# mayuelala/FollowYourClick

Measured on AMD Instinct MI355X. Metric: denoised frames/sec, 16f x 512^2 clip @ 25 DDIM steps, higher is better.
Workload: dtype bf16; 1 GPU; configs[1]: AnimationPipeline DDIM loop, SD-1.5 UNet3D + mm_sd_v15-shaped motion modules (random init), 1 clip/GPU of 16 frames 512x512, 25 DDIM steps, CFG 8.0, mask + first-frame concat, fps/flow conditioning; frames=16, height=512, width=512, ddim_steps=25, parallelism=dp1 (independent clips, weight broadcast 0.00 GiB in 0.00s)

## Files before the change

### followyourclick_amd/_build.py

```python
import concurrent.futures as cf
import hashlib
import os
import shutil
import subprocess
import sys

HERE = os.path.dirname(os.path.abspath(__file__))
CSRC = os.path.join(HERE, "csrc")
EXTRA = os.environ.get("FYC_BUILD_EXTRA", "").split()
LIB = os.path.abspath(os.environ.get("FYC_BUILD_LIB") or os.path.join(HERE, "libfyc_hip.so"))
OBJ = os.path.join(HERE, "_obj") if not (EXTRA or os.environ.get("FYC_BUILD_LIB")) else LIB + ".obj"
SOURCES = ["api.hip", "gemm.hip", "gemm_bf16_plain.hip", "gemm_bf16_conv.hip", "gemm_bf16_act.hip", "gemm_f16_plain.hip", "gemm_f16_conv.hip", "gemm_f16_act.hip", "gemm_f32.hip", "attention.hip", "attention_small.hip", "attention_medium.hip", "attention_large.hip", "attention_small_f16.hip", "attention_medium_f16.hip", "attention_large_f16.hip", "temporal_attn.hip", "temporal_block.hip", "temporal_block_rr.hip", "ff_block.hip", "panel_linear.hip", "norm.hip", "elementwise.hip"]
VARIANTS = os.environ.get("FYC_GEMM_VARIANTS") == "1"
VARIANT_DIR = os.path.join(HERE, "..", "tools", "exp", "gemm_variants")
VARIANT_SOURCES = ["gemm_pp_plain.hip", "gemm_pp_conv.hip", "gemm_ov.hip"] if VARIANTS else []
if VARIANTS:
    EXTRA = EXTRA + ["-DFYC_GEMM_VARIANTS"]
    if not os.environ.get("FYC_BUILD_LIB"):
        raise SystemExit("FYC_GEMM_VARIANTS=1 needs FYC_BUILD_LIB=<path>: the experiment kernels are not part of the product library")
FLAGS = ["--offload-arch=gfx950", "-O3", "-std=c++17", "-fPIC", "-ffp-contract=off", "-Wno-unused-value",
         "-mllvm", "-amdgpu-mfma-vgpr-form=1"]
AGPR_SOURCES = {"ff_block.hip", "panel_linear.hip", "temporal_block_rr.hip"}


NO_SLP_SOURCES = set(filter(None, os.environ.get("FYC_NO_SLP", "ff_block.hip").split(",")))


NO_NAN_SOURCES = {s for s in SOURCES if s.startswith("attention")}


def _flags(src: str):
    fl = FLAGS
    if src in AGPR_SOURCES:
        fl = [f for f in FLAGS if f not in ("-mllvm", "-amdgpu-mfma-vgpr-form=1")]
    if src in NO_SLP_SOURCES:
        fl = fl + ["-fno-slp-vectorize"]
    if src in NO_NAN_SOURCES and os.environ.get("FYC_ATTN_HONOR_NANS") != "1":
        fl = fl + ["-fno-honor-nans"]
    return fl + EXTRA


def _hipcc() -> str:
    for c in (os.environ.get("HIPCC"), shutil.which("hipcc"), "/opt/rocm/bin/hipcc"):
        if c and os.path.exists(c):
            return c
    raise RuntimeError("hipcc not found (need ROCm with gfx950 support)")


def _digest(path: str) -> str:
    h = hashlib.sha256()
    for dep in [path, os.path.join(CSRC, "fyc_common.h"), os.path.join(CSRC, "gemm_kernel.h"), os.path.join(CSRC, "attention_kernel.h"), os.path.join(CSRC, "attention_groups.h"), os.path.join(HERE, "..", "include", "fyc.h")]:
        with open(dep, "rb") as f:
            h.update(f.read())
    h.update(" ".join(_flags(os.path.basename(path))).encode())
    return h.hexdigest()


def source_digest() -> str:
    h = hashlib.sha256()
    files = sorted(f for f in os.listdir(CSRC) if f.endswith((".hip", ".h")))
    for f in files:
        h.update(f.encode())
        with open(os.path.join(CSRC, f), "rb") as fh:
            h.update(fh.read())
    with open(os.path.join(HERE, "..", "include", "fyc.h"), "rb") as fh:
        h.update(fh.read())
    for src in SOURCES:
        h.update((src + " " + " ".join(_flags(src))).encode())
    return h.hexdigest()


def family_digest(family: str = "gemm") -> str:
    if family != "gemm":
        raise ValueError(family)
    h = hashlib.sha256()
    files = sorted(f for f in os.listdir(CSRC) if f.startswith("gemm") and f.endswith((".hip", ".h"))) + ["fyc_common.h"]
    for f in files:
        h.update(f.encode())
        with open(os.path.join(CSRC, f), "rb") as fh:
            h.update(fh.read())
    for src in SOURCES:
        if src.startswith("gemm"):
            h.update((src + " " + " ".join(_flags(src))).encode())
    return h.hexdigest()


def _compile(src: str) -> str:
    path = os.path.join(VARIANT_DIR if src in VARIANT_SOURCES else CSRC, src)
    obj = os.path.join(OBJ, src.replace(".hip", ".o"))
    stamp = obj + ".sha"
    dig = _digest(path)
    if os.path.exists(obj) and os.path.exists(stamp) and open(stamp).read() == dig:
        return obj
    cmd = [_hipcc(), *_flags(src), "-c", path, "-o", obj]
    r = subprocess.run(cmd, capture_output=True, text=True)
    if r.returncode != 0:
        raise RuntimeError(f"hipcc failed for {src}:\n{r.stderr[-4000:]}")
    with open(stamp, "w") as f:
        f.write(dig)
    return obj


def build(force: bool = False, verbose: bool = True) -> str:
    os.makedirs(OBJ, exist_ok=True)
    if force:
        for f in os.listdir(OBJ):
            os.remove(os.path.join(OBJ, f))
    with cf.ThreadPoolExecutor(max_workers=len(SOURCES)) as ex:
        objs = list(ex.map(_compile, SOURCES + VARIANT_SOURCES))
    newest = max(os.path.getmtime(o) for o in objs)
    if force or not os.path.exists(LIB) or os.path.getmtime(LIB) < newest:
        r = subprocess.run([_hipcc(), "--offload-arch=gfx950", "-shared", "-fPIC", "-o", LIB, *objs], capture_output=True, text=True)
        if r.returncode != 0:
            raise RuntimeError(f"link failed:\n{r.stderr[-4000:]}")
    if verbose:
        print(f"[fyc] built {LIB} ({os.path.getsize(LIB) >> 10} KiB)")
    return LIB


if __name__ == "__main__":
    build(force="--force" in sys.argv)
```

### followyourclick_amd/_lib.py

```python
from __future__ import annotations

import ctypes as C
import os

HERE = os.path.dirname(os.path.abspath(__file__))
LIB_PATH = os.environ.get("FYC_LIB_PATH") or os.path.join(HERE, "libfyc_hip.so")

FYC_F32, FYC_BF16, FYC_F16 = 0, 1, 2
GEMM_PLAIN, GEMM_CONV3X3, GEMM_CONV3X3_UP2 = 0, 1, 2
EPI_LINEAR, EPI_GEGLU, EPI_HEADS = 0, 1, 2
ACT_NONE, ACT_GELU, ACT_QUICK_GELU = 0, 1, 2

i32, i64, f32, vp = C.c_int32, C.c_int64, C.c_float, C.c_void_p


class GemmArgs(C.Structure):
    _fields_ = [("a", vp), ("a2", vp), ("w", vp), ("bias", vp), ("rowbias", vp), ("residual", vp), ("out", vp),
                ("seg_out", vp * 3), ("seg_transposed", i32 * 3), ("seg_ld", i32 * 3),
                ("M", i32), ("N", i32), ("K", i32),
                ("lda", i32), ("ldw", i32), ("ldo", i32), ("ldr", i32), ("ldrb", i32), ("k_split", i32), ("lda2", i32),
                ("stride_a", i64), ("stride_w", i64), ("stride_o", i64),
                ("batch", i32), ("mode", i32), ("epilogue", i32),
                ("Hout", i32), ("Wout", i32), ("Hin", i32), ("Win", i32), ("Cin", i32), ("conv_stride", i32), ("conv_pad", i32),
                ("rows_per_batch", i32), ("seg_cols", i32), ("heads", i32), ("tokens", i32),
                ("out_scale", f32), ("dtype", i32), ("tile", i32), ("act", i32), ("ln_stats", vp), ("ln_colsum", vp),
                ("ln_nparts", i32), ("ln_eps", f32), ("chan_parts", vp), ("cs_rows", i32), ("row_parts", vp), ("row_nparts", i32), ("workspace", vp), ("workspace_bytes", i64)]


class AttnArgs(C.Structure):
    _fields_ = [("q", vp), ("k", vp), ("vt", vp), ("o", vp),
                ("batch", i32), ("heads", i32), ("n_q", i32), ("n_k", i32), ("d", i32),
                ("ldo", i32), ("ldvt", i32), ("kv_batch_div", i32), ("o_accumulate", i32),
                ("scale", f32), ("o_scale", f32), ("dtype", i32)]


class TAttnArgs(C.Structure):
    _fields_ = [("qkv", vp), ("o", vp), ("clips", i32), ("frames", i32), ("pixels", i32), ("heads", i32), ("d", i32),
                ("scale", f32), ("dtype", i32)]


class GnStatsArgs(C.Structure):
    _fields_ = [("x", vp), ("stats", vp), ("rows", i32), ("C", i32), ("groups", i32), ("rows_per_sample", i32), ("dtype", i32),
                ("pad_", i32), ("workspace", vp), ("workspace_bytes", i64)]


class GnApplyArgs(C.Structure):
    _fields_ = [("x", vp), ("stats", vp), ("gamma", vp), ("beta", vp), ("y", vp),
                ("rows", i32), ("C", i32), ("groups", i32), ("rows_per_sample", i32), ("eps", f32), ("silu", i32), ("dtype", i32)]


class ChanStatsReduceArgs(C.Structure):
    _fields_ = [("parts", vp), ("cs", vp), ("rows", i32), ("N", i32), ("cs_rows", i32), ("tile_rows", i32), ("slots", i32), ("out_rows", i32)]


class GnApplyCsArgs(C.Structure):
    _fields_ = [("x1", vp), ("cs1", vp), ("x2", vp), ("cs2", vp), ("gamma", vp), ("beta", vp), ("y", vp),
                ("C1", i32), ("C2", i32), ("rows", i32), ("groups", i32), ("rows_per_sample", i32), ("eps", f32), ("silu", i32),
                ("dtype", i32), ("cs_rows", i32)]


class LayerNormArgs(C.Structure):
    _fields_ = [("x", vp), ("gamma", vp), ("beta", vp), ("pe", vp), ("y", vp),
                ("rows", i32), ("C", i32), ("eps", f32), ("pe_div", i32), ("pe_rows", i32), ("dtype", i32)]


class RowStatsArgs(C.Structure):
    _fields_ = [("x", vp), ("stats", vp), ("rows", i32), ("C", i32), ("eps", f32), ("dtype", i32)]


class SoftmaxArgs(C.Structure):
    _fields_ = [("x", vp), ("rows", i64), ("cols", i32), ("ld", i32), ("dtype", i32), ("causal_rows", i32)]


class ConcatArgs(C.Structure):
    _fields_ = [("a", vp), ("b", vp), ("y", vp), ("rows", i64), ("c1", i32), ("c2", i32), ("dtype", i32)]


class SiluArgs(C.Structure):
    _fields_ = [("x", vp), ("y", vp), ("n", i64)]


class CastArgs(C.Structure):
    _fields_ = [("x", vp), ("y", vp), ("rows", i64), ("cols", i32), ("ld", i32), ("dtype", i32)]


class UnetInputArgs(C.Structure):
    _fields_ = [("latents", vp), ("mask", vp), ("first", vp), ("x", vp),
                ("B", i32), ("F", i32), ("HW", i32), ("c_latent", i32), ("c_pad", i32), ("cfg_dup", i32), ("mask_frames", i32),
                ("dtype", i32), ("mode", i32)]


class CfgDdimArgs(C.Structure):
    _fields_ = [("pred", vp), ("latents", vp), ("coef", vp),
                ("B", i32), ("F", i32), ("HW", i32), ("c_latent", i32), ("ld", i32), ("cfg", i32), ("guidance", f32),
                ("pred_type", i32), ("clip_sample", i32), ("dtype", i32), ("pred_single", vp), ("video_scale", f32),
                ("variance_noise", vp), ("sigma", f32), ("clipped_model_output", i32)]


class NchwInArgs(C.Structure):
    _fields_ = [("z", vp), ("x", vp), ("N", i32), ("C", i32), ("HW", i32), ("c_pad", i32), ("scale", f32), ("dtype", i32)]


class NhwcOutArgs(C.Structure):
    _fields_ = [("x", vp), ("y", vp), ("N", i32), ("C", i32), ("HW", i32), ("ld", i32),
                ("mul", f32), ("add", f32), ("lo", f32), ("hi", f32), ("dtype", i32)]


class EmbedArgs(C.Structure):
    _fields_ = [("ids", vp), ("table", vp), ("pos", vp), ("out", vp), ("rows", i64), ("seq", i32), ("C", i32), ("vocab", i32),
                ("dtype", i32)]


class PatchifyArgs(C.Structure):
    _fields_ = [("image", vp), ("out", vp), ("B", i32), ("Cin", i32), ("H", i32), ("W", i32), ("P", i32), ("ld", i32), ("dtype", i32)]


class TemporalBlockArgs(C.Structure):
    _fields_ = [("x", vp), ("out", vp), ("w_qkv", vp), ("colsum", vp), ("bias", vp), ("pe_bias", vp), ("w_out", vp), ("b_out", vp),
                ("clips", i32), ("frames", i32), ("pixels", i32), ("heads", i32), ("d", i32), ("C", i32),
                ("scale", C.c_float), ("eps", C.c_float), ("dtype", i32), ("wstream", vp)]


class FFBlockArgs(C.Structure):
    _fields_ = [("x", vp), ("residual", vp), ("out", vp), ("wstream", vp), ("b_out", vp), ("chan_parts", vp), ("cs_rows", i32),
                ("rows", i32), ("C", i32), ("hidden", i32), ("eps", C.c_float), ("dtype", i32)]


class PanelLinearArgs(C.Structure):
    _fields_ = [("x", vp), ("residual", vp), ("out", vp), ("wstream", vp), ("bias", vp), ("gn_cs", vp), ("gn_gamma", vp), ("gn_beta", vp),
                ("gn_rows_per_sample", i32), ("gn_stat_samples", i32), ("gn_groups", i32), ("gn_eps", C.c_float),
                ("rows", i32), ("N", i32), ("K", i32), ("dtype", i32)]


class PackConv3x3Args(C.Structure):
    _fields_ = [("w", vp), ("out", vp), ("O", i32), ("I", i32), ("dtype", i32)]


class PackGegluArgs(C.Structure):
    _fields_ = [("w", vp), ("b", vp), ("w_out", vp), ("b_out", vp), ("O", i32), ("I", i32), ("dtype", i32)]


OPS = {
    "fyc_gemm": GemmArgs, "fyc_attention": AttnArgs, "fyc_temporal_attention": TAttnArgs,
    "fyc_gn_stats": GnStatsArgs, "fyc_gn_apply": GnApplyArgs, "fyc_layernorm": LayerNormArgs,
    "fyc_softmax_rows": SoftmaxArgs, "fyc_concat_channels": ConcatArgs, "fyc_silu_f32": SiluArgs,
    "fyc_cast_from_f32": CastArgs, "fyc_cast_to_f32": CastArgs, "fyc_unet_input": UnetInputArgs,
    "fyc_cfg_ddim_step": CfgDdimArgs, "fyc_nchw_to_nhwc": NchwInArgs, "fyc_nhwc_to_nchw": NhwcOutArgs,
    "fyc_embed_tokens": EmbedArgs, "fyc_patchify": PatchifyArgs, "fyc_row_stats": RowStatsArgs,
    "fyc_gn_apply_cs": GnApplyCsArgs, "fyc_chan_stats_reduce": ChanStatsReduceArgs,
    "fyc_pack_conv3x3": PackConv3x3Args, "fyc_pack_geglu": PackGegluArgs, "fyc_temporal_block": TemporalBlockArgs,
    "fyc_ff_block": FFBlockArgs, "fyc_panel_linear": PanelLinearArgs,
}
MISC = ["fyc_version", "fyc_last_error", "fyc_init", "fyc_device_caps", "fyc_set_tuning", "fyc_gemm_row_parts", "fyc_gemm_stat_layout", "fyc_gemm_workspace_bytes", "fyc_gn_stats_workspace", "fyc_temporal_block_supported", "fyc_temporal_block_wstream_bytes",
        "fyc_ff_block_supported", "fyc_ff_block_wstream_bytes", "fyc_panel_linear_supported", "fyc_panel_linear_wstream_bytes"]

_lib = None
FYC_VERSION = 301


class FycError(RuntimeError):
    pass


def load() -> C.CDLL:
    global _lib
    if _lib is not None:
        return _lib
    if not os.path.exists(LIB_PATH):
        raise FycError(f"{LIB_PATH} is missing: build it with `python -m followyourclick_amd._build` "
                       "(hipcc --offload-arch=gfx950). There is no CPU fallback.")
    lib = C.CDLL(LIB_PATH)
    lib.fyc_version.restype = C.c_int
    ab_build = bool(os.environ.get("FYC_LIB_PATH"))
    if lib.fyc_version() != FYC_VERSION and not ab_build:
        raise FycError(f"{LIB_PATH} reports ABI version {lib.fyc_version()}, this binding was written against {FYC_VERSION}: argument structs differ "
                       "between major versions - rebuild the library (`python -m followyourclick_amd._build`)")
    lib.fyc_last_error.restype = C.c_char_p
    lib.fyc_init.argtypes = [vp]
    lib.fyc_device_caps.argtypes = [C.POINTER(i64)]
    lib.fyc_set_tuning.argtypes = [C.c_int, C.c_int]
    if not ab_build or hasattr(lib, "fyc_gemm_row_parts"):
        lib.fyc_gemm_row_parts.argtypes = [C.POINTER(GemmArgs)]
        lib.fyc_gemm_row_parts.restype = C.c_int
        lib.fyc_gemm_stat_layout.argtypes = [C.POINTER(GemmArgs), C.POINTER(i32), C.POINTER(i32)]
        lib.fyc_gemm_stat_layout.restype = C.c_int
        lib.fyc_gemm_workspace_bytes.argtypes = [C.POINTER(GemmArgs)]
        lib.fyc_gemm_workspace_bytes.restype = i64
    if not ab_build or hasattr(lib, "fyc_gn_stats_workspace"):
        lib.fyc_gn_stats_workspace.argtypes = [C.POINTER(GnStatsArgs)]
        lib.fyc_gn_stats_workspace.restype = i64
    if not ab_build or hasattr(lib, "fyc_temporal_block_supported"):
        lib.fyc_temporal_block_supported.argtypes = [C.POINTER(TemporalBlockArgs)]
        lib.fyc_temporal_block_supported.restype = C.c_int
    if not ab_build or hasattr(lib, "fyc_temporal_block_wstream_bytes"):
        lib.fyc_temporal_block_wstream_bytes.argtypes = []
        lib.fyc_temporal_block_wstream_bytes.restype = i64
    if not ab_build or hasattr(lib, "fyc_ff_block_supported"):
        lib.fyc_ff_block_supported.argtypes = [C.POINTER(FFBlockArgs)]
        lib.fyc_ff_block_supported.restype = C.c_int
        lib.fyc_ff_block_wstream_bytes.argtypes = []
        lib.fyc_ff_block_wstream_bytes.restype = i64
    if not ab_build or hasattr(lib, "fyc_panel_linear_supported"):
        lib.fyc_panel_linear_supported.argtypes = [C.POINTER(PanelLinearArgs)]
        lib.fyc_panel_linear_supported.restype = C.c_int
        lib.fyc_panel_linear_wstream_bytes.argtypes = [i32, i32]
        lib.fyc_panel_linear_wstream_bytes.restype = i64
    for name, st in OPS.items():
        if ab_build and not hasattr(lib, name):
            continue
        fn = getattr(lib, name)
        fn.argtypes = [C.POINTER(st), vp]
        fn.restype = C.c_int
    _lib = lib
    return lib


def check(rc: int, what: str) -> None:
    if rc != 0:
        raise FycError(f"{what} failed (rc={rc}): {load().fyc_last_error().decode(errors='replace')}")
```

### followyourclick_amd/engine/unet3d.py

```python
from __future__ import annotations

import math
import os
from typing import List, Optional, Sequence, Tuple, Union

import torch

from .. import _lib as L
from .. import ops as ops_mod
from .base import EngineBase
from .config import UNet3DConfig
from .weights import Packed, pack_ff_block, pack_panel_linear, pack_temporal_block

Tensor = torch.Tensor

FUSE_STATS = os.environ.get("FYC_FUSE_STATS", "1") != "0"
FUSE_TEMPORAL = os.environ.get("FYC_FUSE_TEMPORAL", "1") != "0"
TEMPORAL_RR = os.environ.get("FYC_TEMPORAL_RR", "1") != "0"
FUSE_FF = os.environ.get("FYC_FUSE_FF", "1") != "0"
FUSE_PANEL = os.environ.get("FYC_FUSE_PANEL", "1") != "0"
PANEL_ALL = os.environ.get("FYC_PANEL_ALL", "0") != "0"
FUSE_ROWS = os.environ.get("FYC_FUSE_ROWS", "0") != "0"


class Act:
    __slots__ = ("t", "C", "cs", "cs_rows", "rp", "rp_n")

    def __init__(self, t: Tensor, C: int, cs: Optional[Tensor] = None, cs_rows: int = 0, rp: Optional[Tensor] = None, rp_n: int = 0):
        self.t, self.C, self.cs, self.cs_rows, self.rp, self.rp_n = t, C, cs, cs_rows, rp, rp_n


def sinusoid_host(values: Sequence[float], dim: int) -> Tensor:
    half = dim // 2
    v = torch.tensor(list(values), dtype=torch.float32)
    freqs = torch.exp(-math.log(10000.0) * torch.arange(half, dtype=torch.float32) / half)
    ang = v[:, None] * freqs[None, :]
    return torch.cat([torch.cos(ang), torch.sin(ang)], dim=-1).contiguous()


class UNet3DEngine(EngineBase):
    def __init__(self, packed: Packed, ops=None):
        self.P = packed
        self.cfg: UNet3DConfig = packed.cfg
        self.dtype = packed.dtype
        self.ops = ops if ops is not None else ops_mod.get()
        self.device = packed.conv_in_w.device
        self.heads = self.cfg.attention_head_dim
        self.groups = self.cfg.norm_num_groups
        self.mat_attn = self.dtype == torch.float32
        self.transformers: List[Packed] = []
        for blk in self.P.down:
            self.transformers += [l.attn for l in blk.layers if l.attn is not None]
        self.transformers.append(self.P.mid.attn)
        for blk in self.P.up:
            self.transformers += [l.attn for l in blk.layers if l.attn is not None]
        for i, t in enumerate(self.transformers):
            t["idx"] = i
        self.ctx_cache = None
        self.fuse_stats = FUSE_STATS
        self.fuse_rows = FUSE_STATS and FUSE_ROWS
        self.ops.ensure_init(self.device)

    def prepare_time_embeddings(self, timesteps: Sequence[int], fps: Optional[Sequence[float]], flow: Optional[Sequence[float]],
                                batch: int, camera: Optional[Sequence[float]] = None):
        cfg, P, o = self.cfg, self.P, self.ops
        c0, S = cfg.block_out_channels[0], len(timesteps)
        rows = S * batch

        def mlp(m: Packed, sin: Tensor, residual=None) -> Tensor:
            h = self.lin(sin.to(self.device), m.w1, rows, bias=m.b1)
            a = self.new(rows, h.shape[1], dtype=torch.float32)
            o.silu_f32(h, a)
            return self.lin(a, m.w2, rows, bias=m.b2, residual=residual)

        def per_row(v):
            s = sinusoid_host(v, c0)
            return s if s.shape[0] == rows else s.repeat(S, 1)

        emb = mlp(P.emb["time_embedding"], sinusoid_host(timesteps, c0).repeat_interleave(batch, dim=0))
        if cfg.use_camera_motion_condition and camera is not None:
            emb = mlp(P.emb["camera_motion_embedding"], per_row(camera), residual=emb)
        if cfg.use_fps_condition and fps is not None:
            emb = mlp(P.emb["fps_embedding"], per_row(fps), residual=emb)
            emb = mlp(P.emb["motion_embedding"], per_row(flow), residual=emb)
        act = self.new(rows, emb.shape[1], dtype=torch.float32)
        o.silu_f32(emb, act)
        temb = self.lin(act, P.temb_w, rows, bias=P.temb_b)
        return emb, temb

    def prepare_context(self, ctx: Tensor, ip_tokens: Optional[Tensor] = None) -> None:
        cfg, o = self.cfg, self.ops
        Bn, Nk, D = ctx.shape
        H = self.heads

        def to_T(t: Tensor) -> Tensor:
            t = t.to(device=self.device, dtype=torch.float32).contiguous()
            y = self.new(t.shape[0] * t.shape[1], D)
            o.cast_from_f32(t, y, rows=t.shape[0] * t.shape[1], cols=D, ld=D)
            return y

        def project(x: Tensor, w: Tensor, n_tok: int, C: int):
            d = C // H
            ld = ((n_tok + 7) // 8) * 8
            k = self.new(Bn, H, n_tok, d)
            vt = self.zeros(Bn, H, d, ld)
            o.gemm(x, w, None, M=Bn * n_tok, N=2 * C, K=D, lda=D, ldw=D, epilogue=L.EPI_HEADS,
                   heads=dict(seg_cols=C, heads=H, tokens=n_tok, outs=[k, vt], transposed=[0, 1], ld=[0, ld]))
            return k, vt, ld

        if cfg.use_ip_cross_attention and ip_tokens is None:
            n = cfg.ip_num_tokens
            if Nk <= n:
                raise ValueError(f"encoder_hidden_states has {Nk} tokens, the IP cross-attention splits off the last {n}")
            ctx, ip_tokens = ctx[:, :Nk - n], ctx[:, Nk - n:]
            Nk -= n
        xt = to_T(ctx)
        xi = to_T(ip_tokens) if (cfg.use_ip_cross_attention and ip_tokens is not None) else None
        cache = []
        for t in self.transformers:
            e = dict(text=project(xt, t.kv2_w, Nk, t.C), n_text=Nk, ip=None)
            if xi is not None:
                e["ip"] = project(xi, t.kvip_w, ip_tokens.shape[1], t.C)
                e["n_ip"] = ip_tokens.shape[1]
            cache.append(e)
        self.ctx_cache = cache

    def _attend(self, q: Tensor, k: Tensor, vt: Tensor, out: Tensor, *, batch: int, n_q: int, n_k: int, d: int, ldvt: int,
                C: int, kv_div: int, accumulate: bool = False, o_scale: float = 1.0) -> None:
        H, o = self.heads, self.ops
        scale = d ** -0.5
        if not self.mat_attn:
            o.attention(q, k, vt, out, batch=batch, heads=H, n_q=n_q, n_k=n_k, d=d, ldo=C, ldvt=ldvt, scale=scale,
                        kv_batch_div=kv_div, accumulate=accumulate, o_scale=o_scale)
            return
        ldS = ((n_k + 7) // 8) * 8
        for b in range(batch):
            kb = b // kv_div
            S = self.zeros(H, n_q, ldS)
            o.gemm(q[b], k[kb], S, M=n_q, N=n_k, K=d, lda=d, ldw=d, ldo=ldS, batch=H, stride_a=n_q * d, stride_w=n_k * d,
                   stride_o=n_q * ldS, out_scale=scale)
            o.softmax_rows(S, rows=H * n_q, cols=n_k, ld=ldS)
            dst = out[b * n_q:(b + 1) * n_q]
            if accumulate:
                tmp = self.new(n_q, C)
                o.gemm(S, vt[kb], tmp, M=n_q, N=d, K=ldS, lda=ldS, ldw=ldvt, ldo=C, batch=H, stride_a=n_q * ldS, stride_w=d * ldvt,
                       stride_o=d)
                self._axpy(tmp, dst, n_q, C, o_scale)
            else:
                o.gemm(S, vt[kb], dst, M=n_q, N=d, K=ldS, lda=ldS, ldw=ldvt, ldo=C, batch=H, stride_a=n_q * ldS, stride_w=d * ldvt,
                       stride_o=d)

    def row_stats(self, x: Tensor, rows: int, C: int, eps: float = 1e-5) -> Tensor:
        st = self.new(rows, 2, dtype=torch.float32)
        self.ops.row_stats(x, st, rows=rows, C_=C, eps=eps)
        return st

    def _gn(self, x: Union[Act, Tuple[Act, Act]], gamma: Tensor, beta: Tensor, rows: int, rows_per_sample: int, eps: float,
            silu: bool) -> Tuple[Tensor, Optional[Tensor]]:
        o = self.ops
        if isinstance(x, Act):
            if x.cs is not None and rows_per_sample % x.cs_rows == 0:
                y = self.new(rows, x.C)
                o.gn_apply_cs(x.t, x.cs, gamma, beta, y, rows=rows, C1=x.C, groups=self.groups, rows_per_sample=rows_per_sample,
                              eps=eps, silu=silu, cs_rows=x.cs_rows)
                return y, None
            return self.group_norm(x.t, gamma, beta, rows, x.C, rows_per_sample, eps, silu), None
        a, b = x
        if a.cs is not None and b.cs is not None and a.cs_rows == b.cs_rows and rows_per_sample % a.cs_rows == 0:
            y = self.new(rows, a.C + b.C)
            o.gn_apply_cs(a.t, a.cs, gamma, beta, y, rows=rows, C1=a.C, groups=self.groups, rows_per_sample=rows_per_sample,
                          eps=eps, silu=silu, x2=b.t, cs2=b.cs, C2=b.C, cs_rows=a.cs_rows)
            return y, None
        cat = self.new(rows, a.C + b.C)
        o.concat_channels(a.t, b.t, cat, rows=rows, c1=a.C, c2=b.C)
        return self.group_norm(cat, gamma, beta, rows, a.C + b.C, rows_per_sample, eps, silu), cat

    def _lin_rp(self, x: Tensor, w: Tensor, rows: int, bias=None, residual=None) -> Act:
        N, K = w.shape
        out = self.new(rows, N, dtype=x.dtype)
        if FUSE_PANEL and PANEL_ALL and not self.fuse_rows and self.ops.panel_linear_supported(x.dtype, rows=rows, N=N, K=K):
            self.ops.panel_linear(x, out, wstream=self._panel_stream(w), rows=rows, N=N, K=K, bias=bias, residual=residual)
            return Act(out, N)
        rp, n = None, 0
        if self.fuse_rows:
            n = self.ops.gemm_row_parts(x.dtype, M=rows, N=N, K=K)
            rp = self.new(rows, n, 2, dtype=torch.float32)
        self.ops.gemm(x, w, out, M=rows, N=N, K=K, lda=K, ldw=K, ldo=N, bias=bias, residual=residual, ldr=N, row_parts=rp, row_nparts=n)
        return Act(out, N, rp=rp, rp_n=n)

    def _panel_stream(self, w: Tensor) -> Tensor:
        cache = self.__dict__.setdefault("_panel_ws", {})
        key = w.data_ptr()
        hit = cache.get(key)
        if hit is None or hit[0] is not w:
            hit = cache[key] = (w, pack_panel_linear(w))
        return hit[1]

    def _norm_proj_in(self, x: Act, node: Packed, rows: int, rows_per_sample: int) -> Act:
        C = node.C
        if (FUSE_PANEL and isinstance(x, Act) and x.cs is not None and not self.fuse_rows and rows_per_sample % x.cs_rows == 0
                and self.ops.panel_linear_supported(self.dtype, rows=rows, N=C, K=C, gn_rows_per_sample=rows_per_sample, gn_groups=self.groups)):
            out = self.new(rows, C)
            self.ops.panel_linear(x.t, out, wstream=self._panel_stream(node.pin_w), rows=rows, N=C, K=C, bias=node.pin_b, gn_cs=x.cs,
                                  gn_gamma=node.norm_g, gn_beta=node.norm_b, gn_rows_per_sample=rows_per_sample,
                                  gn_stat_samples=rows_per_sample // x.cs_rows, gn_groups=self.groups, gn_eps=1e-6)
            return Act(out, C)
        h, _ = self._gn(x, node.norm_g, node.norm_b, rows, rows_per_sample, 1e-6, False)
        return self._lin_rp(h, node.pin_w, rows, bias=node.pin_b)

    def _ln_args(self, tok: Act, rows: int, C: int) -> dict:
        if tok.rp is not None:
            return dict(ln_stats=tok.rp, ln_nparts=tok.rp_n, ln_eps=1e-5)
        return dict(ln_stats=self.row_stats(tok.t, rows, C))

    def _pe_rowbias(self, a: Packed, B: int, F: int) -> Tensor:
        key = (B, F)
        cache = a.setdefault("_pe_rb", {})
        if key not in cache:
            if F > a.pe_w.shape[0]:
                raise ValueError(f"video_length {F} exceeds the positional table ({a.pe_w.shape[0]})")
            cache[key] = a.pe_w[:F].repeat(B, 1).contiguous()
        return cache[key]

    def _axpy(self, x: Tensor, y: Tensor, rows: int, C: int, alpha: float) -> None:
        key = ("axpy", C, alpha)
        if not hasattr(self, "_eyes"):
            self._eyes = {}
        if key not in self._eyes:
            self._eyes[key] = (torch.eye(C, dtype=torch.float32) * alpha).to(self.dtype).to(self.device)
        self.ops.gemm(x, self._eyes[key], y, M=rows, N=C, K=C, lda=C, ldw=C, ldo=C, residual=y, ldr=C)

    def _conv_act(self, x: Tensor, w: Tensor, b: Tensor, frames: int, Hin: int, Win: int, nxt: Tuple[int, int], **kw) -> Act:
        Cout, K = w.shape
        if kw.get("up2"):
            Ho, Wo = kw["up_size"]
        else:
            st = kw.get("stride", 1)
            Ho, Wo = (Hin - 1) // st + 1, (Win - 1) // st + 1
        rows = frames * Ho * Wo
        plan = self._cs_plan(rows, nxt[0], Cout, K, L.GEMM_CONV3X3_UP2 if kw.get("up2") else L.GEMM_CONV3X3) if nxt else None
        out = self.conv(x, w, b, frames, Hin, Win, chan_parts=None if plan is None else plan[0], cs_rows=nxt[0] if plan is not None else 0, **kw)
        return Act(out, Cout, None if plan is None else self._cs_finish(plan, rows, nxt[0], Cout, nxt[1]), nxt[1] if nxt else 0)

    def resnet(self, r: Packed, x: Union[Act, Tuple[Act, Act]], temb: Tensor, g: dict, nxt: Tuple[int, int]) -> Act:
        rows, rpb = g["rows"], g["F"] * g["H"] * g["W"]
        frames = g["B"] * g["F"]
        h, cat = self._gn(x, r.n1_g, r.n1_b, rows, rpb, self.cfg.norm_eps, True)
        tb = temb[:, r.temb_off:]
        h1 = self._conv_act(h, r.c1_w, r.c1_b, frames, g["H"], g["W"], (g["H"] * g["W"], rpb), rowbias=tb,
                            rpb=g["H"] * g["W"] if g.get("temb_per_frame") else rpb, ldrb=temb.shape[1])
        h2, _ = self._gn(h1, r.n2_g, r.n2_b, rows, rpb, self.cfg.norm_eps, True)
        if r.sc_w is None:
            sc = x.t
        elif isinstance(x, Act) or cat is not None:
            sc = self.lin(cat if cat is not None else x.t, r.sc_w, rows, bias=r.sc_b)
        else:
            a, b = x
            sc = self.new(rows, r.cout)
            self.ops.gemm(a.t, r.sc_w, sc, M=rows, N=r.cout, K=a.C + b.C, lda=a.C, ldw=a.C + b.C, ldo=r.cout, bias=r.sc_b,
                          a2=b.t, k_split=a.C, lda2=b.C)
        return self._conv_act(h2, r.c2_w, r.c2_b, frames, g["H"], g["W"], nxt, residual=sc)

    def feed_forward_out(self, ff: Packed, ln, tok: Act, residual: Optional[Tensor], rows: int, C: int, nxt=None) -> Act:
        hidden = ff.w1.shape[0] // 2
        cs_rows = nxt[0] if (nxt and self.fuse_stats) else 0
        fused = FUSE_FF and ff.cs1 is not None
        if fused and cs_rows and not self.ops.ff_block_supported(self.dtype, rows=rows, C_=C, hidden=hidden, cs_rows=cs_rows):
            cs_rows = 0
        if fused and self.ops.ff_block_supported(self.dtype, rows=rows, C_=C, hidden=hidden, cs_rows=cs_rows):
            if "_wstream" not in ff:
                ff["_wstream"] = pack_ff_block(ff)
            out = self.new(rows, C)
            parts = self.new(rows // 128 * C * 2, dtype=torch.float32) if cs_rows else None
            self.ops.ff_block(tok.t, residual, out, wstream=ff["_wstream"], b_out=ff.po_b, rows=rows, C_=C, hidden=hidden,
                              chan_parts=parts, cs_rows=cs_rows)
            cs = self._cs_finish((parts, 128, 1), rows, nxt[0], C, nxt[1]) if cs_rows else None
            return Act(out, C, cs, nxt[1] if cs_rows else 0)
        if ff.cs1 is not None:
            N1 = ff.w1.shape[0]
            hmid = self.new(rows, N1 // 2)
            self.ops.gemm(tok.t, ff.w1, hmid, M=rows, N=N1, K=C, lda=C, ldw=C, ldo=N1 // 2, bias=ff.b1, epilogue=L.EPI_GEGLU,
                          ln_colsum=ff.cs1, **self._ln_args(tok, rows, C))
        else:
            n = self.layer_norm(tok.t, ln, rows, C)
            hmid = self.lin(n, ff.w1, rows, bias=ff.b1, geglu=True)
        out = self.new(rows, C)
        K = ff.po_w.shape[1]
        plan = self._cs_plan(rows, nxt[0], C, K, L.GEMM_PLAIN) if nxt else None
        rp, rp_n = None, 0
        if residual is None and self.fuse_rows:
            rp_n = self.ops.gemm_row_parts(tok.t.dtype, M=rows, N=C, K=K)
            rp = self.new(rows, rp_n, 2, dtype=torch.float32)
        self.ops.gemm(tok.t, ff.po_w, out, M=rows, N=C, K=K, lda=C, ldw=K, ldo=C, bias=ff.po_b, residual=residual, ldr=C,
                      a2=hmid, k_split=C, lda2=K - C, chan_parts=None if plan is None else plan[0], cs_rows=nxt[0] if plan is not None else 0,
                      row_parts=rp, row_nparts=rp_n)
        return Act(out, C, None if plan is None else self._cs_finish(plan, rows, nxt[0], C, nxt[1]), nxt[1] if nxt else 0, rp, rp_n)

    def transformer(self, t: Packed, x: Act, g: dict, nxt: Tuple[int, int]) -> Act:
        rows, C, H, o = g["rows"], t.C, self.heads, self.ops
        BF, N = g["B"] * g["F"], g["H"] * g["W"]
        d = C // H
        tok = self._norm_proj_in(x, t, rows, N)
        ld = ((N + 7) // 8) * 8
        q, k, vt = self.new(BF, H, N, d), self.new(BF, H, N, d), (self.zeros(BF, H, d, ld) if ld != N else self.new(BF, H, d, ld))
        hd = dict(seg_cols=C, heads=H, tokens=N, outs=[q, k, vt], transposed=[0, 0, 1], ld=[0, 0, ld])
        if t.qkv_f is not None:
            w, b, cs = t.qkv_f
            o.gemm(tok.t, w, None, M=rows, N=3 * C, K=C, lda=C, ldw=C, bias=b, epilogue=L.EPI_HEADS, heads=hd, ln_colsum=cs,
                   **self._ln_args(tok, rows, C))
        else:
            n1 = self.layer_norm(tok.t, t.ln1, rows, C)
            o.gemm(n1, t.qkv_w, None, M=rows, N=3 * C, K=C, lda=C, ldw=C, epilogue=L.EPI_HEADS, heads=hd)
        att = self.new(rows, C)
        self._attend(q, k, vt, att, batch=BF, n_q=N, n_k=N, d=d, ldvt=ld, C=C, kv_div=1)
        tok = self._lin_rp(att, t.o1_w, rows, bias=t.o1_b, residual=tok.t)
        q2 = self.new(BF, H, N, d)
        hd2 = dict(seg_cols=C, heads=H, tokens=N, outs=[q2], transposed=[0], ld=[0])
        if t.q2_f is not None:
            w, b, cs = t.q2_f
            o.gemm(tok.t, w, None, M=rows, N=C, K=C, lda=C, ldw=C, bias=b, epilogue=L.EPI_HEADS, heads=hd2, ln_colsum=cs,
                   **self._ln_args(tok, rows, C))
        else:
            n2 = self.layer_norm(tok.t, t.ln2, rows, C)
            o.gemm(n2, t.q2_w, None, M=rows, N=C, K=C, lda=C, ldw=C, epilogue=L.EPI_HEADS, heads=hd2)
        cache = self.ctx_cache[t.idx]
        kt, vtt, ldt = cache["text"]
        att2 = self.new(rows, C)
        self._attend(q2, kt, vtt, att2, batch=BF, n_q=N, n_k=cache["n_text"], d=d, ldvt=ldt, C=C, kv_div=g["F"])
        if cache["ip"] is not None:
            ki, vti, ldi = cache["ip"]
            self._attend(q2, ki, vti, att2, batch=BF, n_q=N, n_k=cache["n_ip"], d=d, ldvt=ldi, C=C, kv_div=g["F"],
                         accumulate=True, o_scale=self.cfg.ip_scale)
        tok = self._lin_rp(att2, t.o2_w, rows, bias=t.o2_b, residual=tok.t)
        return self.feed_forward_out(t.ff, t.ln3, tok, x.t, rows, C, nxt)

    def motion(self, m: Packed, x: Act, g: dict, nxt: Tuple[int, int]) -> Act:
        rows, C, o = g["rows"], m.C, self.ops
        N, Hm = g["H"] * g["W"], self.cfg.motion_num_attention_heads
        d = C // Hm
        tok = self._norm_proj_in(x, m, rows, N)
        for bi, blk in enumerate(m.blocks):
            for a in blk.attns:
                if FUSE_TEMPORAL and a.qkv_f is not None and o.temporal_block_supported(self.dtype, clips=g["B"], frames=g["F"], pixels=N, heads=Hm, d=d):
                    cache = a.setdefault("_tblock", {})
                    if g["F"] not in cache:
                        cache[g["F"]] = pack_temporal_block(a, Hm, g["F"])
                    out = self.new(rows, C)
                    kw = cache[g["F"]]
                    if not TEMPORAL_RR and "wstream" in kw:
                        kw = {k: v for k, v in kw.items() if k != "wstream"}
                    o.temporal_block(tok.t, out, clips=g["B"], frames=g["F"], pixels=N, heads=Hm, d=d, scale=d ** -0.5, **kw)
                    tok = Act(out, C)
                    continue
                if a.qkv_f is not None:
                    w, b, cs = a.qkv_f
                    qkv = self.new(rows, 3 * C)
                    rb = self._pe_rowbias(a, g["B"], g["F"]) if a.pe_w is not None else None
                    o.gemm(tok.t, w, qkv, M=rows, N=3 * C, K=C, lda=C, ldw=C, ldo=3 * C, bias=b, rowbias=rb, rows_per_batch=N,
                           ln_colsum=cs, **self._ln_args(tok, rows, C))
                else:
                    n = self.layer_norm(tok.t, a.ln, rows, C, pe=a.pe, pe_div=N, pe_rows=g["F"])
                    qkv = self.lin(n, a.qkv_w, rows)
                att = self.new(rows, C)
                o.temporal_attention(qkv, att, clips=g["B"], frames=g["F"], pixels=N, heads=Hm, d=d, scale=d ** -0.5)
                tok = self._lin_rp(att, a.o_w, rows, bias=a.o_b, residual=tok.t)
            last = bi == len(m.blocks) - 1
            tok = self.feed_forward_out(blk.ff, blk.ff_ln, tok, x.t if last else None, rows, C, nxt if last else None)
        return tok

    def forward(self, x: Tensor, temb: Tensor, B: int, F: int, H: int, W: int, temb_first: Optional[Tensor] = None) -> Tensor:
        assert self.ctx_cache is not None, "call prepare_context() first"
        cfg, P = self.cfg, self.P
        g = dict(B=B, F=F, H=H, W=W, rows=B * F * H * W)
        if temb_first is not None:
            temb = temb.repeat_interleave(F, dim=0)
            temb[0::F] = temb_first
            g["temb_per_frame"] = True
        frames = B * F

        def hw(gg):
            return gg["H"] * gg["W"]

        def frame(gg):
            return hw(gg), hw(gg)

        def clip(gg):
            return hw(gg), F * hw(gg)

        def layer(l, xin, gg):
            y = self.resnet(l.resnet, xin, temb, gg, frame(gg) if (l.attn is not None or l.motion is not None) else clip(gg))
            if l.attn is not None:
                y = self.transformer(l.attn, y, gg, frame(gg) if l.motion is not None else clip(gg))
            if l.motion is not None:
                y = self.motion(l.motion, y, gg, clip(gg))
            return y

        x = self._conv_act(x, P.conv_in_w, P.conv_in_b, frames, H, W, clip(g))
        skips = [x]
        sizes = [(H, W)]
        for blk in P.down:
            for l in blk.layers:
                x = layer(l, x, g)
                skips.append(x)
            if blk.down is not None:
                g2 = dict(g, H=(g["H"] - 1) // 2 + 1, W=(g["W"] - 1) // 2 + 1)
                g2["rows"] = B * F * g2["H"] * g2["W"]
                x = self._conv_act(x.t, blk.down.w, blk.down.b, frames, g["H"], g["W"], clip(g2), stride=2)
                g = g2
                sizes.append((g["H"], g["W"]))
                skips.append(x)
        x = self.resnet(P.mid.r0, x, temb, g, frame(g))
        x = self.transformer(P.mid.attn, x, g, frame(g) if P.mid.motion is not None else clip(g))
        if P.mid.motion is not None:
            x = self.motion(P.mid.motion, x, g, clip(g))
        x = self.resnet(P.mid.r1, x, temb, g, clip(g))
        for blk in P.up:
            for l in blk.layers:
                x = layer(l, (x, skips.pop()), g)
            if blk.up is not None:
                sizes.pop()
                Hn, Wn = sizes[-1]
                g2 = dict(g, H=Hn, W=Wn)
                g2["rows"] = B * F * Hn * Wn
                x = self._conv_act(x.t, blk.up.w, blk.up.b, frames, g["H"], g["W"], clip(g2), up2=True, up_size=(Hn, Wn))
                g = g2
        h, _ = self._gn(x, P.out_g, P.out_b, g["rows"], F * hw(g), cfg.norm_eps, True)
        return self.conv(h, P.conv_out_w, P.conv_out_b, frames, g["H"], g["W"])
```

### followyourclick_amd/engine/weights.py

```python
from __future__ import annotations

import os

from typing import Dict, Optional

import torch

from .config import UNet3DConfig, VAEDecoderConfig

Tensor = torch.Tensor
K_ALIGN = 64


def pad_channels(c: int) -> int:
    return ((c + K_ALIGN - 1) // K_ALIGN) * K_ALIGN


def conv_slab(dtype) -> int:
    return 128 // torch.empty((), dtype=dtype).element_size()


def pack_conv3x3(w: Tensor, dtype, device) -> Tensor:
    O, I, kh, kw = w.shape
    assert kh == 3 and kw == 3
    Ip, sl = pad_channels(I), conv_slab(dtype)
    p = torch.zeros(O, Ip, 3, 3, dtype=torch.float32)
    p[:, :I] = w
    p = p.reshape(O, Ip // sl, sl, 3, 3).permute(0, 1, 3, 4, 2)
    return p.reshape(O, 9 * Ip).to(dtype).contiguous().to(device)


def pack_linear(w: Tensor, dtype, device, k_pad: Optional[int] = None) -> Tensor:
    w = w.reshape(w.shape[0], -1)
    if k_pad is not None and k_pad != w.shape[1]:
        p = torch.zeros(w.shape[0], k_pad, dtype=torch.float32)
        p[:, : w.shape[1]] = w
        w = p
    return w.to(dtype).contiguous().to(device)


def pack_geglu(w: Tensor, b: Tensor, dtype, device):
    O, I = w.shape
    half = O // 2
    assert half % 16 == 0
    wv, wg = w[:half].reshape(half // 16, 16, I), w[half:].reshape(half // 16, 16, I)
    bv, bg = b[:half].reshape(half // 16, 16), b[half:].reshape(half // 16, 16)
    wp = torch.stack([wv, wg], dim=1).reshape(O, I)
    bp = torch.stack([bv, bg], dim=1).reshape(O)
    return wp.to(dtype).contiguous().to(device), bp.float().contiguous().to(device)


def f32(t: Tensor, device) -> Tensor:
    return t.detach().float().contiguous().to(device)


def fold_layernorm(w: Tensor, b: Optional[Tensor], gamma: Tensor, beta: Tensor, dtype, device, geglu: bool = False):
    w = w.reshape(w.shape[0], -1).double()
    wf = (w * gamma.double()[None, :]).float()
    bias = (w @ beta.double() + (b.double() if b is not None else 0.0)).float()
    if geglu:
        wp, bp = pack_geglu(wf, bias, dtype, device)
    else:
        wp, bp = pack_linear(wf, dtype, device), f32(bias, device)
    return wp, bp, wp.float().sum(dim=1).contiguous()

LN_FOLD = os.environ.get("FYC_LN_FOLD", "1") != "0"


class Packed(dict):
    __getattr__ = dict.__getitem__


def _resnet(sd: Dict[str, Tensor], p: str, dtype, device, temb: bool = True) -> Packed:
    r = Packed(
        n1_g=f32(sd[p + ".norm1.weight"], device), n1_b=f32(sd[p + ".norm1.bias"], device),
        c1_w=pack_conv3x3(sd[p + ".conv1.weight"], dtype, device), c1_b=f32(sd[p + ".conv1.bias"], device),
        n2_g=f32(sd[p + ".norm2.weight"], device), n2_b=f32(sd[p + ".norm2.bias"], device),
        c2_w=pack_conv3x3(sd[p + ".conv2.weight"], dtype, device), c2_b=f32(sd[p + ".conv2.bias"], device),
        cin=sd[p + ".conv1.weight"].shape[1], cout=sd[p + ".conv1.weight"].shape[0], sc_w=None, sc_b=None)
    if (p + ".conv_shortcut.weight") in sd:
        r["sc_w"] = pack_linear(sd[p + ".conv_shortcut.weight"], dtype, device)
        r["sc_b"] = f32(sd[p + ".conv_shortcut.bias"], device)
    return r


def _ff(sd, p, dtype, device, proj_out_w: Tensor, proj_out_b: Tensor, ln: Optional[str] = None) -> Packed:
    cs1 = None
    if ln is not None and LN_FOLD:
        w1, b1, cs1 = fold_layernorm(sd[p + ".net.0.proj.weight"], sd[p + ".net.0.proj.bias"], sd[ln + ".weight"], sd[ln + ".bias"],
                                     dtype, device, geglu=True)
    else:
        w1, b1 = pack_geglu(sd[p + ".net.0.proj.weight"], sd[p + ".net.0.proj.bias"], dtype, device)
    w2, b2 = sd[p + ".net.2.weight"].double(), sd[p + ".net.2.bias"].double()
    wp, bp = proj_out_w.reshape(proj_out_w.shape[0], -1).double(), proj_out_b.double()
    merged_w = torch.cat([wp, wp @ w2], dim=1).float()
    merged_b = (bp + wp @ b2).float()
    return Packed(w1=w1, b1=b1, cs1=cs1, po_w=pack_linear(merged_w, dtype, device), po_b=f32(merged_b, device))


def _ln(sd, p, device):
    return f32(sd[p + ".weight"], device), f32(sd[p + ".bias"], device)


def _transformer(sd, p: str, cfg: UNet3DConfig, dtype, device) -> Packed:
    t = p + ".transformer_blocks.0"
    a1, a2 = t + ".attn1", t + ".attn2"
    d = Packed(
        C=sd[p + ".proj_in.weight"].shape[0],
        norm_g=f32(sd[p + ".norm.weight"], device), norm_b=f32(sd[p + ".norm.bias"], device),
        pin_w=pack_linear(sd[p + ".proj_in.weight"], dtype, device), pin_b=f32(sd[p + ".proj_in.bias"], device),
        ln1=_ln(sd, t + ".norm1", device), ln2=_ln(sd, t + ".norm2", device), ln3=_ln(sd, t + ".norm3", device),
        qkv_w=pack_linear(torch.cat([sd[a1 + ".to_q.weight"], sd[a1 + ".to_k.weight"], sd[a1 + ".to_v.weight"]], 0), dtype, device),
        o1_w=pack_linear(sd[a1 + ".to_out.0.weight"], dtype, device), o1_b=f32(sd[a1 + ".to_out.0.bias"], device),
        q2_w=pack_linear(sd[a2 + ".to_q.weight"], dtype, device),
        kv2_w=pack_linear(torch.cat([sd[a2 + ".to_k.weight"], sd[a2 + ".to_v.weight"]], 0), dtype, device),
        o2_w=pack_linear(sd[a2 + ".to_out.0.weight"], dtype, device), o2_b=f32(sd[a2 + ".to_out.0.bias"], device),
        ff=_ff(sd, t + ".ff", dtype, device, sd[p + ".proj_out.weight"], sd[p + ".proj_out.bias"], ln=t + ".norm3"), kvip_w=None,
        qkv_f=None, q2_f=None)
    if LN_FOLD:
        qkv = torch.cat([sd[a1 + ".to_q.weight"], sd[a1 + ".to_k.weight"], sd[a1 + ".to_v.weight"]], 0)
        d["qkv_f"] = fold_layernorm(qkv, None, sd[t + ".norm1.weight"], sd[t + ".norm1.bias"], dtype, device)
        d["q2_f"] = fold_layernorm(sd[a2 + ".to_q.weight"], None, sd[t + ".norm2.weight"], sd[t + ".norm2.bias"], dtype, device)
        d["qkv_w"] = d["q2_w"] = None
    if cfg.use_ip_cross_attention:
        d["kvip_w"] = pack_linear(torch.cat([sd[a2 + ".to_k_ip.weight"], sd[a2 + ".to_v_ip.weight"]], 0), dtype, device)
    return d


def _motion(sd, p: str, cfg: UNet3DConfig, dtype, device) -> Packed:
    p = p + ".temporal_transformer"
    C = sd[p + ".proj_in.weight"].shape[0]
    blocks = []
    for b in range(cfg.motion_num_transformer_block):
        t = f"{p}.transformer_blocks.{b}"
        attns = []
        for a in range(cfg.motion_attention_blocks):
            ab = f"{t}.attention_blocks.{a}"
            pe = None
            if cfg.temporal_position_encoding:
                pe = sinusoidal_pe(C, max(cfg.temporal_position_encoding_max_len, 32)).to(device)
            qkv = torch.cat([sd[ab + ".to_q.weight"], sd[ab + ".to_k.weight"], sd[ab + ".to_v.weight"]], 0)
            att = Packed(ln=_ln(sd, f"{t}.norms.{a}", device), pe=pe, qkv_w=None, qkv_f=None, pe_w=None,
                         o_w=pack_linear(sd[ab + ".to_out.0.weight"], dtype, device), o_b=f32(sd[ab + ".to_out.0.bias"], device))
            if LN_FOLD:
                att["qkv_f"] = fold_layernorm(qkv, None, sd[f"{t}.norms.{a}.weight"], sd[f"{t}.norms.{a}.bias"], dtype, device)
                if pe is not None:
                    att["pe_w"] = (pe.double().cpu() @ qkv.double().t()).float().contiguous().to(device)
            else:
                att["qkv_w"] = pack_linear(qkv, dtype, device)
            attns.append(att)
        last = b == cfg.motion_num_transformer_block - 1
        if last:
            ff = _ff(sd, t + ".ff", dtype, device, sd[p + ".proj_out.weight"], sd[p + ".proj_out.bias"], ln=t + ".ff_norm")
        else:
            ff = _ff(sd, t + ".ff", dtype, device, torch.eye(C), torch.zeros(C), ln=t + ".ff_norm")
        blocks.append(Packed(attns=attns, ff_ln=_ln(sd, t + ".ff_norm", device), ff=ff))
    return Packed(C=C, norm_g=f32(sd[p + ".norm.weight"], device), norm_b=f32(sd[p + ".norm.bias"], device),
                  pin_w=pack_linear(sd[p + ".proj_in.weight"], dtype, device), pin_b=f32(sd[p + ".proj_in.bias"], device),
                  blocks=blocks)


def pack_temporal_block(att: Packed, heads: int, frames: int) -> dict:
    w, b, cs = att.qkv_f
    C = w.shape[1]
    d = C // heads
    assert 3 * d <= 128 and d <= 48

    def per_head(t: Tensor) -> Tensor:
        out = torch.zeros(heads, 128, *t.shape[1:], dtype=t.dtype, device=t.device)
        for i in range(3):
            out[:, i * d:(i + 1) * d] = t[i * C:(i + 1) * C].reshape(heads, d, *t.shape[1:])
        return out.contiguous()

    pe = None
    if att.pe_w is not None:
        if frames > att.pe_w.shape[0]:
            raise ValueError(f"video_length {frames} exceeds the positional table ({att.pe_w.shape[0]})")
        pe = per_head(att.pe_w[:frames].t().contiguous()).permute(2, 0, 1).contiguous()
    wo = torch.zeros(heads, C, 48, dtype=att.o_w.dtype, device=att.o_w.device)
    wo[:, :, :d] = att.o_w.reshape(C, heads, d).permute(1, 0, 2)
    ops = dict(w_qkv=per_head(w), colsum=per_head(cs), bias=per_head(b), pe_bias=pe, w_out=wo.contiguous(), b_out=att.o_b)
    if frames == 16 and C % 32 == 0:
        ops["wstream"] = pack_temporal_stream(ops["w_qkv"], ops["bias"], pe, ops["w_out"], d)
    return ops


def temporal_block_layout(C: int) -> dict:
    ks, nb = C // 32, C // 16
    lay = dict(ks=ks, nb=nb, a_tab=6 * ks, a_pieces=6 * ks + 6, b_wo=3 * ks, b_tab=3 * ks + 2 * nb, b_pieces=3 * ks + 2 * nb + 3)
    lay["stride"] = max(lay["a_pieces"], lay["b_pieces"])
    return lay


def temporal_slot_feature(t: int, k: int) -> int:
    g, e = k // 8, k % 8
    if t == 0:
        return 4 * g + e if e < 4 else 16 + 4 * g + e - 4
    return 32 + 4 * g + e if e < 4 else 48


def pack_temporal_stream(w_qkv: Tensor, bias: Tensor, pe_bias: Optional[Tensor], w_out: Tensor, d: int) -> Tensor:
    H, _, C = w_qkv.shape
    F = 16
    assert d <= 48 and C % 32 == 0 and (pe_bias is None or pe_bias.shape[0] == F)
    lay = temporal_block_layout(C)
    ks, nb = lay["ks"], lay["nb"]
    T, dev = w_qkv.dtype, w_qkv.device
    st = torch.zeros(2 * H, lay["stride"], 512, dtype=T, device=dev)
    qkv = torch.zeros(H, 3, 48, C, dtype=T, device=dev)
    for i in range(3):
        qkv[:, i, :d] = w_qkv[:, i * d:(i + 1) * d]
    blk = qkv[:, :2].reshape(H, 2, 3, 16, ks, 32).permute(0, 4, 1, 2, 3, 5).reshape(H, ks * 6, 16, 32)
    st[0::2, :6 * ks] = _mfma_fragments(blk)
    tb = bias.float()[:, None, :] + (pe_bias.float().permute(1, 0, 2) if pe_bias is not None else 0.0)
    tb = tb.expand(H, F, 128)
    ta = torch.zeros(H, F, 96, dtype=torch.float32, device=dev)
    ta[:, :, :d] = tb[:, :, :d]
    ta[:, :, 48:48 + d] = tb[:, :, d:2 * d]
    st[0::2, lay["a_tab"]:lay["a_tab"] + 6] = ta.reshape(H, -1).contiguous().view(T).reshape(H, 6, 512)
    blk = qkv[:, 2].reshape(H, 3, 16, ks, 32).permute(0, 3, 1, 2, 4).reshape(H, ks * 3, 16, 32)
    st[1::2, :3 * ks] = _mfma_fragments(blk)
    slot = torch.tensor([[temporal_slot_feature(t, k) for k in range(32)] for t in range(2)], device=dev)
    wo_ext = torch.cat([w_out, torch.zeros(H, C, 1, dtype=w_out.dtype, device=dev)], dim=2)
    wog = wo_ext[:, :, slot.reshape(-1)].reshape(H, nb, 16, 2, 32).permute(0, 3, 1, 2, 4).reshape(H, 2 * nb, 16, 32)
    st[1::2, lay["b_wo"]:lay["b_wo"] + 2 * nb] = _mfma_fragments(wog.to(T))
    tv = torch.zeros(H, 48, F, dtype=torch.float32, device=dev)
    tv[:, :d] = tb[:, :, 2 * d:3 * d].transpose(1, 2)
    st[1::2, lay["b_tab"]:lay["b_tab"] + 3] = tv.reshape(H, -1).contiguous().view(T).reshape(H, 3, 512)
    return st.reshape(-1).contiguous()


def ff_block_layout(C: int, hidden: int):
    nb, ks, chunks = C // 32, C // 16, hidden // 32
    sa = (7 * ks + 9) // 10
    hp = max(2 * nb, 2 * sa + 1, 2 * (ks - sa) + 2 * nb)
    return ks // 2 + 2 * chunks + 2, (hp + 3) // 4 * 4, sa


def ff_slot_unit(sg: int, k: int) -> int:
    kh, e = k // 8, k % 8
    return 16 * sg + 8 * (e // 4) + 4 * kh + e % 4


def _mfma_fragments32(w: Tensor) -> Tensor:
    lead = w.shape[:-2]
    return w.reshape(*lead, 32, 2, 8).transpose(-3, -2).reshape(*lead, 512)


def _mfma_fragments(w: Tensor) -> Tensor:
    lead = w.shape[:-2]
    return w.reshape(*lead, 16, 4, 8).transpose(-3, -2).reshape(*lead, 512)


def pack_ff_block(ff: Packed) -> Tensor:
    w1, b1, po = ff.w1, ff.b1, ff.po_w
    assert ff.cs1 is not None, "fyc_ff_block needs the LayerNorm folded into FF1"
    C = w1.shape[1]
    hid = w1.shape[0] // 2
    assert C % 32 == 0 and hid % 32 == 0 and tuple(po.shape) == (C, C + hid) and w1.dtype == po.dtype
    nb, ks, chunks = C // 32, C // 16, hid // 32
    nh, hp, sa = ff_block_layout(C, hid)
    npj = ks // 2
    dev = w1.device
    st = torch.zeros(nh, hp, 512, dtype=w1.dtype, device=dev)
    wp = _mfma_fragments32(po[:, :C].reshape(nb, 32, npj, 2, 16).permute(2, 3, 0, 1, 4))
    st[:npj, : 2 * nb] = wp.reshape(npj, 2 * nb, 512)
    vg = w1.reshape(chunks, 2, 2, 16, C).permute(0, 2, 1, 3, 4).reshape(chunks, 2, 32, C)
    f1 = _mfma_fragments32(vg.reshape(chunks, 2, 32, ks, 16).permute(0, 3, 1, 2, 4))
    ha = torch.arange(chunks, device=dev) * 2 + npj
    st[ha, : 2 * sa] = f1[:, :sa].reshape(chunks, 2 * sa, 512)
    st[ha + 1, : 2 * (ks - sa)] = f1[:, sa:].reshape(chunks, 2 * (ks - sa), 512)
    cst = torch.zeros(chunks, 512 * w1.element_size() // 4, dtype=torch.float32, device=dev)
    cst[:, :64] = b1.reshape(chunks, 2, 2, 16).permute(0, 2, 1, 3).reshape(chunks, 64)
    st[ha + 2, 2 * sa] = cst.view(w1.dtype)
    slot = torch.tensor([[ff_slot_unit(sg, k) for k in range(16)] for sg in range(2)], device=dev)
    w2 = po[:, C:].reshape(nb, 32, chunks, 32)[..., slot.reshape(-1)].reshape(nb, 32, chunks, 2, 16)
    f2 = _mfma_fragments32(w2.permute(2, 3, 0, 1, 4))
    st[ha + 3, 2 * (ks - sa): 2 * (ks - sa) + 2 * nb] = f2.reshape(chunks, 2 * nb, 512)
    return st.reshape(-1).contiguous()


def pack_panel_linear(w: Tensor) -> Tensor:
    N, K = w.shape
    pn = min(N, 320)
    assert N % pn == 0 and pn % 16 == 0 and K % 64 == 0
    fr = _mfma_fragments(w.reshape(N // pn, pn // 16, 16, K // 64, 2, 32).permute(0, 3, 4, 1, 2, 5))
    return fr.reshape(-1).contiguous()


def sinusoidal_pe(channels: int, length: int) -> Tensor:
    import math
    pos = torch.arange(length, dtype=torch.float32)[:, None]
    div = torch.exp(torch.arange(0, channels, 2, dtype=torch.float32) * (-math.log(10000.0) / channels))
    pe = torch.zeros(length, channels)
    pe[:, 0::2] = torch.sin(pos * div)
    pe[:, 1::2] = torch.cos(pos * div)
    return pe.contiguous()


def pack_unet(sd: Dict[str, Tensor], cfg: UNet3DConfig, dtype, device) -> Packed:
    cfg.validate()
    sd = {k: v.detach().float().cpu() for k, v in sd.items()}
    nb = len(cfg.block_out_channels)
    P = Packed(cfg=cfg, dtype=dtype)
    half = 0.5 if cfg.use_first_frame_condition_concat else 1.0
    P["conv_in_w"] = pack_conv3x3(sd["conv_in.weight"] * half, dtype, device)
    P["conv_in_b"] = f32(sd["conv_in.bias"] * half, device)
    emb = {}
    for name in (["time_embedding"] + (["camera_motion_embedding"] if cfg.use_camera_motion_condition else [])
                 + (["fps_embedding", "motion_embedding"] if cfg.use_fps_condition else [])):
        emb[name] = Packed(w1=f32(sd[name + ".linear_1.weight"], device), b1=f32(sd[name + ".linear_1.bias"], device),
                           w2=f32(sd[name + ".linear_2.weight"], device), b2=f32(sd[name + ".linear_2.bias"], device))
    P["emb"] = emb
    resnets, temb_w, temb_b = [], [], []

    def add_resnet(p):
        r = _resnet(sd, p, dtype, device)
        r["temb_off"] = sum(w.shape[0] for w in temb_w)
        temb_w.append(sd[p + ".time_emb_proj.weight"])
        temb_b.append(sd[p + ".time_emb_proj.bias"])
        resnets.append(r)
        return r

    down = []
    for i, bt in enumerate(cfg.down_block_types):
        p = f"down_blocks.{i}"
        layers = []
        for j in range(cfg.layers_per_block):
            layers.append(Packed(
                resnet=add_resnet(f"{p}.resnets.{j}"),
                attn=_transformer(sd, f"{p}.attentions.{j}", cfg, dtype, device) if bt.startswith("CrossAttn") else None,
                motion=_motion(sd, f"{p}.motion_modules.{j}", cfg, dtype, device)
                if cfg.use_motion_module and (2 ** i) in cfg.motion_module_resolutions else None))
        ds = None
        if i != nb - 1:
            ds = Packed(w=pack_conv3x3(sd[f"{p}.downsamplers.0.conv.weight"], dtype, device), b=f32(sd[f"{p}.downsamplers.0.conv.bias"], device))
        down.append(Packed(layers=layers, down=ds))
    P["down"] = down
    P["mid"] = Packed(r0=add_resnet("mid_block.resnets.0"), attn=_transformer(sd, "mid_block.attentions.0", cfg, dtype, device),
                      motion=_motion(sd, "mid_block.motion_modules.0", cfg, dtype, device)
                      if cfg.use_motion_module and cfg.motion_module_mid_block else None,
                      r1=add_resnet("mid_block.resnets.1"))
    up = []
    for i, bt in enumerate(cfg.up_block_types):
        p = f"up_blocks.{i}"
        layers = []
        for j in range(cfg.layers_per_block + 1):
            layers.append(Packed(
                resnet=add_resnet(f"{p}.resnets.{j}"),
                attn=_transformer(sd, f"{p}.attentions.{j}", cfg, dtype, device) if bt.startswith("CrossAttn") else None,
                motion=_motion(sd, f"{p}.motion_modules.{j}", cfg, dtype, device)
                if cfg.use_motion_module and (2 ** (nb - 1 - i)) in cfg.motion_module_resolutions else None))
        us = None
        if i != nb - 1:
            us = Packed(w=pack_conv3x3(sd[f"{p}.upsamplers.0.conv.weight"], dtype, device), b=f32(sd[f"{p}.upsamplers.0.conv.bias"], device))
        up.append(Packed(layers=layers, up=us))
    P["up"] = up
    P["out_g"], P["out_b"] = f32(sd["conv_norm_out.weight"], device), f32(sd["conv_norm_out.bias"], device)
    P["conv_out_w"] = pack_conv3x3(sd["conv_out.weight"], dtype, device)
    P["conv_out_b"] = f32(sd["conv_out.bias"], device)
    P["temb_w"] = f32(torch.cat(temb_w, 0), device)
    P["temb_b"] = f32(torch.cat(temb_b, 0), device)
    P["temb_total"] = P["temb_w"].shape[0]
    return P


def pack_vae_decoder(sd: Dict[str, Tensor], cfg: VAEDecoderConfig, dtype, device) -> Packed:
    sd = {k: v.detach().float().cpu() for k, v in sd.items()}
    P = Packed(cfg=cfg, dtype=dtype)
    P["pq_w"] = pack_linear(sd["post_quant_conv.weight"], dtype, device, k_pad=pad_channels(cfg.latent_channels))
    P["pq_b"] = f32(sd["post_quant_conv.bias"], device)
    P["conv_in_w"] = pack_conv3x3(sd["decoder.conv_in.weight"], dtype, device)
    P["conv_in_b"] = f32(sd["decoder.conv_in.bias"], device)
    P["mid_r0"] = _resnet(sd, "decoder.mid_block.resnets.0", dtype, device)
    a = "decoder.mid_block.attentions.0"
    P["attn"] = Packed(g=f32(sd[a + ".group_norm.weight"], device), b=f32(sd[a + ".group_norm.bias"], device),
                       qkv_w=pack_linear(torch.cat([sd[a + ".query.weight"], sd[a + ".key.weight"], sd[a + ".value.weight"]], 0), dtype, device),
                       qkv_b=f32(torch.cat([sd[a + ".query.bias"], sd[a + ".key.bias"], sd[a + ".value.bias"]], 0), device),
                       o_w=pack_linear(sd[a + ".proj_attn.weight"], dtype, device), o_b=f32(sd[a + ".proj_attn.bias"], device))
    P["mid_r1"] = _resnet(sd, "decoder.mid_block.resnets.1", dtype, device)
    ups = []
    nb = len(cfg.block_out_channels)
    for i in range(nb):
        rs = [_resnet(sd, f"decoder.up_blocks.{i}.resnets.{j}", dtype, device) for j in range(cfg.layers_per_block + 1)]
        us = None
        if i != nb - 1:
            k = f"decoder.up_blocks.{i}.upsamplers.0.conv"
            us = Packed(w=pack_conv3x3(sd[k + ".weight"], dtype, device), b=f32(sd[k + ".bias"], device))
        ups.append(Packed(resnets=rs, up=us))
    P["ups"] = ups
    P["out_g"], P["out_b"] = f32(sd["decoder.conv_norm_out.weight"], device), f32(sd["decoder.conv_norm_out.bias"], device)
    P["conv_out_w"] = pack_conv3x3(sd["decoder.conv_out.weight"], dtype, device)
    P["conv_out_b"] = f32(sd["decoder.conv_out.bias"], device)
    return P


def _vae_attn(sd, a: str, dtype, device) -> Packed:
    return Packed(g=f32(sd[a + ".group_norm.weight"], device), b=f32(sd[a + ".group_norm.bias"], device),
                  qkv_w=pack_linear(torch.cat([sd[a + ".query.weight"], sd[a + ".key.weight"], sd[a + ".value.weight"]], 0), dtype, device),
                  qkv_b=f32(torch.cat([sd[a + ".query.bias"], sd[a + ".key.bias"], sd[a + ".value.bias"]], 0), device),
                  o_w=pack_linear(sd[a + ".proj_attn.weight"], dtype, device), o_b=f32(sd[a + ".proj_attn.bias"], device))


def pack_vae_encoder(sd: Dict[str, Tensor], cfg: VAEDecoderConfig, dtype, device) -> Packed:
    sd = {k: v.detach().float().cpu() for k, v in sd.items()}
    P = Packed(cfg=cfg, dtype=dtype)
    P["conv_in_w"] = pack_conv3x3(sd["encoder.conv_in.weight"], dtype, device)
    P["conv_in_b"] = f32(sd["encoder.conv_in.bias"], device)
    downs = []
    nb = len(cfg.block_out_channels)
    for i in range(nb):
        rs = [_resnet(sd, f"encoder.down_blocks.{i}.resnets.{j}", dtype, device) for j in range(cfg.layers_per_block)]
        ds = None
        if i != nb - 1:
            k = f"encoder.down_blocks.{i}.downsamplers.0.conv"
            ds = Packed(w=pack_conv3x3(sd[k + ".weight"], dtype, device), b=f32(sd[k + ".bias"], device))
        downs.append(Packed(resnets=rs, down=ds))
    P["downs"] = downs
    P["mid_r0"] = _resnet(sd, "encoder.mid_block.resnets.0", dtype, device)
    P["attn"] = _vae_attn(sd, "encoder.mid_block.attentions.0", dtype, device)
    P["mid_r1"] = _resnet(sd, "encoder.mid_block.resnets.1", dtype, device)
    P["out_g"], P["out_b"] = f32(sd["encoder.conv_norm_out.weight"], device), f32(sd["encoder.conv_norm_out.bias"], device)
    P["conv_out_w"] = pack_conv3x3(sd["encoder.conv_out.weight"], dtype, device)
    P["conv_out_b"] = f32(sd["encoder.conv_out.bias"], device)
    C2 = 2 * cfg.latent_channels
    P["q_w"] = pack_linear(sd["quant_conv.weight"], dtype, device, k_pad=pad_channels(C2))
    P["q_b"] = f32(sd["quant_conv.bias"], device)
    return P
```

### followyourclick_amd/ops.py

```python
from __future__ import annotations

import os

import ctypes as C
from typing import Optional

import torch

from . import _lib as L

Tensor = torch.Tensor


_DTYPE_CODES = {torch.bfloat16: L.FYC_BF16, torch.float16: L.FYC_F16, torch.float32: L.FYC_F32}


def _dtc(dtype: torch.dtype) -> int:
    try:
        return _DTYPE_CODES[dtype]
    except KeyError:
        raise TypeError(f"unsupported activation dtype {dtype}") from None


def _dt(t: Tensor) -> int:
    return _dtc(t.dtype)


def _p(t: Optional[Tensor]) -> Optional[int]:
    if t is None:
        return None
    if not t.is_cuda:
        raise L.FycError("followyourclick_amd ops need HIP device tensors; there is no CPU fallback")
    return t.data_ptr()


def _f32(t: Optional[Tensor], what: str) -> Optional[int]:
    if t is not None and t.dtype != torch.float32:
        raise TypeError(f"{what} must be float32")
    return _p(t)


_raw_stream = getattr(torch._C, "_cuda_getCurrentRawStream", None) or (lambda idx: torch.cuda.current_stream(idx).cuda_stream)


class HipOps:

    name = "hip"

    def __init__(self):
        self.lib = L.load()
        self._zero = None
        self._ws = None
        self._ws_need = {}
        self._q_cache = {}
        self._inited_dev = None

    def ensure_init(self, device: torch.device) -> None:
        if self._inited_dev is not None and getattr(device, "index", None) == self._inited_dev:
            return
        if not torch.cuda.is_available():
            raise L.FycError("no HIP device visible: followyourclick_amd has no CPU fallback")
        device = torch.device(device)
        idx = device.index if device.index is not None else torch.cuda.current_device()
        if self._inited_dev == idx:
            return
        if self._inited_dev is not None:
            raise L.FycError(f"followyourclick_amd is bound to cuda:{self._inited_dev}; use one process per GPU (asked for cuda:{idx})")
        self._zero = torch.zeros(4096, dtype=torch.uint8, device=torch.device("cuda", idx))
        L.check(self.lib.fyc_init(self._zero.data_ptr()), "fyc_init")
        self.abi_version = int(self.lib.fyc_version())
        self._inited_dev = idx
        for kv in filter(None, os.environ.get("FYC_TUNING", "").split(",")):
            k, v = kv.split("=")
            self.set_tuning(int(k), int(v))

    def device_caps(self):
        caps = (L.i64 * 8)()
        L.check(self.lib.fyc_device_caps(caps), "fyc_device_caps")
        return list(caps)

    def set_tuning(self, key: int, value: int) -> None:
        L.check(self.lib.fyc_set_tuning(key, value), "fyc_set_tuning")
        self._ws_need.clear()
        self._q_cache.clear()

    def _stream(self) -> int:
        return _raw_stream(self._inited_dev if self._inited_dev is not None else torch.cuda.current_device())

    def _call(self, name: str, args) -> None:
        L.check(getattr(self.lib, name)(C.byref(args), self._stream()), name)

    def gemm(self, a: Tensor, w: Tensor, out: Optional[Tensor], *, M: int, N: int, K: int, lda: int, ldw: int,
             ldo: int = 0, bias: Optional[Tensor] = None, rowbias: Optional[Tensor] = None, rows_per_batch: int = 1,
             residual: Optional[Tensor] = None, ldr: int = 0, ldrb: int = 0, out_scale: float = 1.0, epilogue: int = L.EPI_LINEAR,
             mode: int = L.GEMM_PLAIN, conv: Optional[dict] = None, batch: int = 1, stride_a: int = 0,
             stride_w: int = 0, stride_o: int = 0, heads: Optional[dict] = None, tile: int = 0,
             a2: Optional[Tensor] = None, k_split: int = 0, lda2: int = 0, act: int = L.ACT_NONE,
             ln_stats: Optional[Tensor] = None, ln_colsum: Optional[Tensor] = None, ln_nparts: int = 0, ln_eps: float = 1e-5,
             chan_parts: Optional[Tensor] = None, cs_rows: int = 0, row_parts: Optional[Tensor] = None, row_nparts: int = 0) -> None:
        self.ensure_init(a.device)
        g = self._gemm_args(a, w, out, M=M, N=N, K=K, lda=lda, ldw=ldw, ldo=ldo, bias=bias, rowbias=rowbias, rows_per_batch=rows_per_batch,
                            residual=residual, ldr=ldr, ldrb=ldrb, out_scale=out_scale, epilogue=epilogue, mode=mode, conv=conv, batch=batch,
                            stride_a=stride_a, stride_w=stride_w, stride_o=stride_o, heads=heads, tile=tile, a2=a2, k_split=k_split,
                            lda2=lda2, act=act, ln_stats=ln_stats, ln_colsum=ln_colsum, ln_nparts=ln_nparts, ln_eps=ln_eps,
                            chan_parts=chan_parts, cs_rows=cs_rows, row_parts=row_parts, row_nparts=row_nparts)
        key = (M, N, K, mode, epilogue, act, batch, tile, g.dtype, ln_stats is not None, chan_parts is not None, row_parts is not None)
        need = self._ws_need.get(key)
        if need is None:
            need = int(self.lib.fyc_gemm_workspace_bytes(C.byref(g))) if hasattr(self.lib, "fyc_gemm_workspace_bytes") else 0
            self._ws_need[key] = need
        if need > 0:
            if self._ws is None or self._ws.numel() < need or self._ws.device != a.device:
                self._ws = torch.empty(need, dtype=torch.uint8, device=a.device)
            g.workspace, g.workspace_bytes = self._ws.data_ptr(), self._ws.numel()
        self._call("fyc_gemm", g)

    def gemm_row_parts(self, dtype: torch.dtype, *, M: int, N: int, K: int, mode: int = L.GEMM_PLAIN, batch: int = 1, tile: int = 0) -> int:
        key = ("rp", dtype, M, N, K, mode, batch, tile)
        if key not in self._q_cache:
            g = L.GemmArgs()
            g.M, g.N, g.K, g.mode, g.batch, g.tile = M, N, K, mode, batch, tile
            g.dtype = _dtc(dtype)
            self._q_cache[key] = int(self.lib.fyc_gemm_row_parts(C.byref(g))) if hasattr(self.lib, "fyc_gemm_row_parts") else 0
        return self._q_cache[key]

    def gemm_split_bytes(self, dtype: torch.dtype, *, M: int, N: int, K: int, mode: int = L.GEMM_PLAIN) -> int:
        key = ("sb", dtype, M, N, K, mode)
        if key not in self._q_cache:
            g = L.GemmArgs()
            g.M, g.N, g.K, g.mode, g.batch, g.epilogue = M, N, K, mode, 1, L.EPI_LINEAR
            g.dtype = _dtc(dtype)
            self._q_cache[key] = int(self.lib.fyc_gemm_workspace_bytes(C.byref(g))) if hasattr(self.lib, "fyc_gemm_workspace_bytes") else 0
        return self._q_cache[key]

    def gemm_stat_layout(self, dtype: torch.dtype, *, M: int, N: int, K: int, cs_rows: int, mode: int = L.GEMM_PLAIN, batch: int = 1,
                         tile: int = 0):
        key = ("sl", dtype, M, N, K, cs_rows, mode, batch, tile)
        if key not in self._q_cache:
            if not hasattr(self.lib, "fyc_gemm_stat_layout"):
                self._q_cache[key] = (0, 0, 0)
            else:
                g = L.GemmArgs()
                g.M, g.N, g.K, g.mode, g.batch, g.tile, g.cs_rows = M, N, K, mode, batch, tile, cs_rows
                g.dtype = _dtc(dtype)
                tr, sl = L.i32(0), L.i32(0)
                n = int(self.lib.fyc_gemm_stat_layout(C.byref(g), C.byref(tr), C.byref(sl)))
                self._q_cache[key] = (n, int(tr.value), int(sl.value))
        return self._q_cache[key]

    def chan_stats_reduce(self, parts: Tensor, cs: Tensor, *, rows: int, N: int, cs_rows: int, tile_rows: int, slots: int,
                          out_rows: int = 0) -> None:
        if cs.dtype != torch.float64:
            raise TypeError("channel statistics must be float64")
        a = L.ChanStatsReduceArgs()
        a.parts, a.cs, a.rows, a.N, a.cs_rows, a.tile_rows, a.slots = _f32(parts, "parts"), _p(cs), rows, N, cs_rows, tile_rows, slots
        a.out_rows = out_rows
        self._call("fyc_chan_stats_reduce", a)

    @staticmethod
    def _gemm_args(a, w, out, *, M, N, K, lda, ldw, ldo, bias, rowbias, rows_per_batch, residual, ldr, ldrb, out_scale, epilogue, mode,
                   conv, batch, stride_a, stride_w, stride_o, heads, tile, a2, k_split, lda2, act, ln_stats, ln_colsum, ln_nparts,
                   ln_eps, chan_parts, cs_rows, row_parts, row_nparts):
        g = L.GemmArgs()
        g.a, g.w, g.bias, g.rowbias = _p(a), _p(w), _f32(bias, "bias"), _f32(rowbias, "rowbias")
        g.residual, g.out = _p(residual), _p(out)
        g.M, g.N, g.K, g.lda, g.ldw, g.ldo, g.ldr, g.ldrb = M, N, K, lda, ldw, ldo, ldr, ldrb
        g.stride_a, g.stride_w, g.stride_o, g.batch = stride_a, stride_w, stride_o, batch
        g.mode, g.epilogue, g.rows_per_batch, g.out_scale, g.dtype = mode, epilogue, rows_per_batch, out_scale, _dt(a)
        g.tile, g.act = tile, act
        g.ln_stats, g.ln_colsum = _f32(ln_stats, "ln_stats"), _f32(ln_colsum, "ln_colsum")
        g.a2, g.k_split, g.lda2 = _p(a2), k_split, lda2
        if a.dtype != w.dtype:
            raise TypeError(f"gemm: activation {a.dtype} vs weight {w.dtype}")
        if conv is not None:
            g.Hout, g.Wout, g.Hin, g.Win, g.Cin, g.conv_stride = (conv["Hout"], conv["Wout"], conv["Hin"], conv["Win"],
                                                                  conv["Cin"], conv.get("stride", 1))
            g.conv_pad = conv.get("pad", 1)
        if heads is not None:
            g.seg_cols, g.heads, g.tokens = heads["seg_cols"], heads["heads"], heads["tokens"]
            for i, (t, tr, ld) in enumerate(zip(heads["outs"], heads["transposed"], heads["ld"])):
                g.seg_out[i], g.seg_transposed[i], g.seg_ld[i] = _p(t), int(tr), int(ld)
        g.ln_nparts, g.ln_eps = ln_nparts, ln_eps
        g.chan_parts, g.cs_rows = _f32(chan_parts, "chan_parts"), cs_rows
        g.row_parts, g.row_nparts = _f32(row_parts, "row_parts"), row_nparts
        return g

    def attention(self, q: Tensor, k: Tensor, vt: Tensor, o: Tensor, *, batch: int, heads: int, n_q: int, n_k: int,
                  d: int, ldo: int, ldvt: int, scale: float, kv_batch_div: int = 1, accumulate: bool = False,
                  o_scale: float = 1.0) -> None:
        self.ensure_init(q.device)
        a = L.AttnArgs()
        a.q, a.k, a.vt, a.o = _p(q), _p(k), _p(vt), _p(o)
        a.batch, a.heads, a.n_q, a.n_k, a.d, a.ldo, a.ldvt = batch, heads, n_q, n_k, d, ldo, ldvt
        a.kv_batch_div, a.o_accumulate, a.scale, a.o_scale, a.dtype = kv_batch_div, int(accumulate), scale, o_scale, _dt(q)
        self._call("fyc_attention", a)

    def temporal_attention(self, qkv: Tensor, o: Tensor, *, clips: int, frames: int, pixels: int, heads: int, d: int,
                           scale: float) -> None:
        self.ensure_init(qkv.device)
        a = L.TAttnArgs()
        a.qkv, a.o, a.clips, a.frames, a.pixels, a.heads, a.d, a.scale, a.dtype = (_p(qkv), _p(o), clips, frames, pixels,
                                                                                  heads, d, scale, _dt(qkv))
        self._call("fyc_temporal_attention", a)

    def _tblock_args(self, x, out, w_qkv, colsum, bias, pe_bias, w_out, b_out, clips, frames, pixels, heads, d, scale, eps):
        a = L.TemporalBlockArgs()
        a.x, a.out, a.w_qkv, a.w_out = _p(x), _p(out), _p(w_qkv), _p(w_out)
        a.colsum, a.bias, a.pe_bias, a.b_out = _f32(colsum, "colsum"), _f32(bias, "bias"), _f32(pe_bias, "pe_bias"), _f32(b_out, "b_out")
        a.clips, a.frames, a.pixels, a.heads, a.d, a.C = clips, frames, pixels, heads, d, heads * d
        a.scale, a.eps, a.dtype = scale, eps, _dt(x)
        return a

    def temporal_block_supported(self, dtype: torch.dtype, *, clips: int, frames: int, pixels: int, heads: int, d: int) -> bool:
        if not hasattr(self.lib, "fyc_temporal_block_supported"):
            return False
        a = L.TemporalBlockArgs()
        a.clips, a.frames, a.pixels, a.heads, a.d, a.C = clips, frames, pixels, heads, d, heads * d
        a.dtype = _dtc(dtype)
        return bool(self.lib.fyc_temporal_block_supported(C.byref(a)))

    def temporal_block(self, x: Tensor, out: Tensor, *, w_qkv: Tensor, colsum: Tensor, bias: Tensor, pe_bias: Optional[Tensor],
                       w_out: Tensor, b_out: Tensor, clips: int, frames: int, pixels: int, heads: int, d: int, scale: float,
                       eps: float = 1e-5, wstream: Optional[Tensor] = None) -> None:
        self.ensure_init(x.device)
        a = self._tblock_args(x, out, w_qkv, colsum, bias, pe_bias, w_out, b_out, clips, frames, pixels, heads, d, scale, eps)
        if wstream is not None and hasattr(self.lib, "fyc_temporal_block_wstream_bytes"):
            if "tbw" not in self._q_cache:
                self._q_cache["tbw"] = int(self.lib.fyc_temporal_block_wstream_bytes())
            if wstream.numel() * wstream.element_size() != self._q_cache["tbw"]:
                raise ValueError(f"temporal_block: wstream has {wstream.numel() * wstream.element_size()} bytes, expected {self._q_cache['tbw']}")
            a.wstream = _p(wstream)
        self._call("fyc_temporal_block", a)

    def ff_block_supported(self, dtype: torch.dtype, *, rows: int, C_: int, hidden: int, cs_rows: int = 0) -> bool:
        if not hasattr(self.lib, "fyc_ff_block_supported"):
            return False
        key = ("ffs", dtype, rows, C_, hidden, cs_rows)
        if key in self._q_cache:
            return self._q_cache[key]
        a = L.FFBlockArgs()
        a.rows, a.C, a.hidden, a.cs_rows = rows, C_, hidden, cs_rows
        a.chan_parts = 16 if cs_rows > 0 else None
        a.dtype = _dtc(dtype)
        self._q_cache[key] = bool(self.lib.fyc_ff_block_supported(C.byref(a)))
        return self._q_cache[key]

    def ff_block_wstream_bytes(self) -> int:
        if "ffw" not in self._q_cache:
            self._q_cache["ffw"] = int(self.lib.fyc_ff_block_wstream_bytes())
        return self._q_cache["ffw"]

    def ff_block(self, x: Tensor, residual: Optional[Tensor], out: Tensor, *, wstream: Tensor, b_out: Tensor, rows: int, C_: int,
                 hidden: int, eps: float = 1e-5, chan_parts: Optional[Tensor] = None, cs_rows: int = 0) -> None:
        self.ensure_init(x.device)
        if wstream.numel() * wstream.element_size() != self.ff_block_wstream_bytes():
            raise ValueError(f"ff_block: wstream has {wstream.numel() * wstream.element_size()} bytes, expected {self.ff_block_wstream_bytes()}")
        a = L.FFBlockArgs()
        a.x, a.residual, a.out, a.wstream, a.b_out = _p(x), _p(residual), _p(out), _p(wstream), _f32(b_out, "b_out")
        a.chan_parts, a.cs_rows = _f32(chan_parts, "chan_parts"), cs_rows
        a.rows, a.C, a.hidden, a.eps, a.dtype = rows, C_, hidden, eps, _dt(x)
        self._call("fyc_ff_block", a)

    def panel_linear_supported(self, dtype: torch.dtype, *, rows: int, N: int, K: int, gn_rows_per_sample: int = 0, gn_groups: int = 32) -> bool:
        if not hasattr(self.lib, "fyc_panel_linear_supported"):
            return False
        key = ("pls", dtype, rows, N, K, gn_rows_per_sample, gn_groups)
        if key not in self._q_cache:
            a = L.PanelLinearArgs()
            a.rows, a.N, a.K = rows, N, K
            a.dtype = _dtc(dtype)
            if gn_rows_per_sample > 0:
                a.gn_cs, a.gn_rows_per_sample, a.gn_stat_samples, a.gn_groups = 16, gn_rows_per_sample, 1, gn_groups
            self._q_cache[key] = bool(self.lib.fyc_panel_linear_supported(C.byref(a)))
        return self._q_cache[key]

    def panel_linear(self, x: Tensor, out: Tensor, *, wstream: Tensor, rows: int, N: int, K: int, bias: Optional[Tensor] = None,
                     residual: Optional[Tensor] = None, gn_cs: Optional[Tensor] = None, gn_gamma: Optional[Tensor] = None,
                     gn_beta: Optional[Tensor] = None, gn_rows_per_sample: int = 0, gn_stat_samples: int = 1, gn_groups: int = 32,
                     gn_eps: float = 1e-6) -> None:
        self.ensure_init(x.device)
        key = ("plw", N, K)
        if key not in self._q_cache:
            self._q_cache[key] = int(self.lib.fyc_panel_linear_wstream_bytes(N, K))
        need = self._q_cache[key]
        if wstream.numel() * wstream.element_size() != need:
            raise ValueError(f"panel_linear: wstream has {wstream.numel() * wstream.element_size()} bytes, expected {need}")
        if gn_cs is not None and gn_cs.dtype != torch.float64:
            raise TypeError("panel_linear: gn_cs must be float64")
        a = L.PanelLinearArgs()
        a.x, a.residual, a.out, a.wstream, a.bias = _p(x), _p(residual), _p(out), _p(wstream), _f32(bias, "bias")
        a.gn_cs, a.gn_gamma, a.gn_beta = _p(gn_cs), _f32(gn_gamma, "gn_gamma"), _f32(gn_beta, "gn_beta")
        a.gn_rows_per_sample, a.gn_stat_samples, a.gn_groups, a.gn_eps = gn_rows_per_sample, gn_stat_samples, gn_groups, gn_eps
        a.rows, a.N, a.K, a.dtype = rows, N, K, _dt(x)
        self._call("fyc_panel_linear", a)

    def gn_stats(self, x: Tensor, stats: Tensor, *, rows: int, C_: int, groups: int, rows_per_sample: int) -> None:
        a = L.GnStatsArgs()
        if stats.dtype != torch.float64:
            raise TypeError("gn stats buffer must be float64")
        a.x, a.stats, a.rows, a.C, a.groups, a.rows_per_sample, a.dtype = _p(x), _p(stats), rows, C_, groups, rows_per_sample, _dt(x)
        key = ("gnws", rows, groups, rows_per_sample)
        need = self._q_cache.get(key)
        if need is None:
            need = self._q_cache[key] = int(self.lib.fyc_gn_stats_workspace(C.byref(a))) if hasattr(self.lib, "fyc_gn_stats_workspace") else 0
        if need > 0:
            if self._ws is None or self._ws.numel() < need or self._ws.device != x.device:
                self._ws = torch.empty(need, dtype=torch.uint8, device=x.device)
            a.workspace, a.workspace_bytes = self._ws.data_ptr(), self._ws.numel()
        self._call("fyc_gn_stats", a)

    def gn_apply(self, x: Tensor, stats: Tensor, gamma: Tensor, beta: Tensor, y: Tensor, *, rows: int, C_: int,
                 groups: int, rows_per_sample: int, eps: float, silu: bool) -> None:
        a = L.GnApplyArgs()
        a.x, a.stats, a.gamma, a.beta, a.y = _p(x), _p(stats), _f32(gamma, "gamma"), _f32(beta, "beta"), _p(y)
        a.rows, a.C, a.groups, a.rows_per_sample, a.eps, a.silu, a.dtype = rows, C_, groups, rows_per_sample, eps, int(silu), _dt(x)
        self._call("fyc_gn_apply", a)

    def gn_apply_cs(self, x1: Tensor, cs1: Tensor, gamma: Tensor, beta: Tensor, y: Tensor, *, rows: int, C1: int, groups: int,
                    rows_per_sample: int, eps: float, silu: bool, x2: Optional[Tensor] = None, cs2: Optional[Tensor] = None,
                    C2: int = 0, cs_rows: int = 0) -> None:
        a = L.GnApplyCsArgs()
        for t in (cs1, cs2):
            if t is not None and t.dtype != torch.float64:
                raise TypeError("channel statistics must be float64")
        a.x1, a.cs1, a.x2, a.cs2 = _p(x1), _p(cs1), _p(x2), _p(cs2)
        a.gamma, a.beta, a.y = _f32(gamma, "gamma"), _f32(beta, "beta"), _p(y)
        a.C1, a.C2, a.rows, a.groups, a.rows_per_sample, a.eps, a.silu, a.dtype = C1, C2, rows, groups, rows_per_sample, eps, int(silu), _dt(x1)
        a.cs_rows = cs_rows
        self._call("fyc_gn_apply_cs", a)

    def layernorm(self, x: Tensor, gamma: Tensor, beta: Tensor, y: Tensor, *, rows: int, C_: int, eps: float = 1e-5,
                  pe: Optional[Tensor] = None, pe_div: int = 1, pe_rows: int = 1) -> None:
        a = L.LayerNormArgs()
        a.x, a.gamma, a.beta, a.pe, a.y = _p(x), _f32(gamma, "gamma"), _f32(beta, "beta"), _f32(pe, "pe"), _p(y)
        a.rows, a.C, a.eps, a.pe_div, a.pe_rows, a.dtype = rows, C_, eps, pe_div, pe_rows, _dt(x)
        self._call("fyc_layernorm", a)

    def row_stats(self, x: Tensor, stats: Tensor, *, rows: int, C_: int, eps: float = 1e-5) -> None:
        a = L.RowStatsArgs()
        a.x, a.stats, a.rows, a.C, a.eps, a.dtype = _p(x), _f32(stats, "stats"), rows, C_, eps, _dt(x)
        self._call("fyc_row_stats", a)

    def softmax_rows(self, x: Tensor, *, rows: int, cols: int, ld: int, causal_rows: int = 0) -> None:
        a = L.SoftmaxArgs()
        a.x, a.rows, a.cols, a.ld, a.dtype, a.causal_rows = _p(x), rows, cols, ld, _dt(x), causal_rows
        self._call("fyc_softmax_rows", a)

    def concat_channels(self, a_: Tensor, b_: Tensor, y: Tensor, *, rows: int, c1: int, c2: int) -> None:
        a = L.ConcatArgs()
        a.a, a.b, a.y, a.rows, a.c1, a.c2, a.dtype = _p(a_), _p(b_), _p(y), rows, c1, c2, _dt(a_)
        self._call("fyc_concat_channels", a)

    def embed_tokens(self, ids: Tensor, table: Tensor, pos: Tensor, out: Tensor, *, rows: int, seq: int, C_: int) -> None:
        if ids.dtype != torch.int64 or table.dtype != torch.float32 or pos.dtype != torch.float32:
            raise TypeError("embed_tokens: ids must be int64, tables float32")
        a = L.EmbedArgs()
        a.ids, a.table, a.pos, a.out = _p(ids), _p(table), _p(pos), _p(out)
        a.rows, a.seq, a.C, a.vocab, a.dtype = rows, seq, C_, table.shape[0], _dt(out)
        self._call("fyc_embed_tokens", a)

    def patchify(self, image: Tensor, out: Tensor, *, B: int, Cin: int, H: int, W: int, P: int, ld: int) -> None:
        if image.dtype != torch.float32:
            raise TypeError("patchify: image must be float32 NCHW")
        a = L.PatchifyArgs()
        a.image, a.out, a.B, a.Cin, a.H, a.W, a.P, a.ld, a.dtype = _p(image), _p(out), B, Cin, H, W, P, ld, _dt(out)
        self._call("fyc_patchify", a)

    def pack_conv3x3(self, w: Tensor, out: Tensor) -> None:
        a = L.PackConv3x3Args()
        a.w, a.out, a.O, a.I, a.dtype = _f32(w, "w"), _p(out), w.shape[0], w.shape[1], _dt(out)
        self._call("fyc_pack_conv3x3", a)

    def pack_geglu(self, w: Tensor, b: Optional[Tensor], w_out: Tensor, b_out: Optional[Tensor]) -> None:
        a = L.PackGegluArgs()
        a.w, a.b, a.w_out, a.b_out = _f32(w, "w"), _f32(b, "b"), _p(w_out), _f32(b_out, "b_out")
        a.O, a.I, a.dtype = w.shape[0], w.shape[1], _dt(w_out)
        self._call("fyc_pack_geglu", a)

    def silu_f32(self, x: Tensor, y: Tensor) -> None:
        a = L.SiluArgs()
        a.x, a.y, a.n = _f32(x, "x"), _f32(y, "y"), x.numel()
        self._call("fyc_silu_f32", a)

    def cast_from_f32(self, x: Tensor, y: Tensor, *, rows: int, cols: int, ld: int) -> None:
        a = L.CastArgs()
        a.x, a.y, a.rows, a.cols, a.ld, a.dtype = _f32(x, "x"), _p(y), rows, cols, ld, _dt(y)
        self._call("fyc_cast_from_f32", a)

    def cast_to_f32(self, x: Tensor, y: Tensor, *, rows: int, cols: int, ld: int) -> None:
        a = L.CastArgs()
        a.x, a.y, a.rows, a.cols, a.ld, a.dtype = _p(x), _f32(y, "y"), rows, cols, ld, _dt(x)
        self._call("fyc_cast_to_f32", a)

    def unet_input(self, latents: Tensor, mask: Optional[Tensor], first: Optional[Tensor], x: Tensor, *, B: int, F: int,
                   HW: int, c_latent: int, c_pad: int, cfg_dup: int, mask_frames: int = 1, mode: int = 0) -> None:
        self.ensure_init(latents.device)
        a = L.UnetInputArgs()
        a.latents, a.mask, a.first, a.x = _f32(latents, "latents"), _f32(mask, "mask"), _f32(first, "first"), _p(x)
        a.B, a.F, a.HW, a.c_latent, a.c_pad, a.cfg_dup, a.mask_frames, a.dtype, a.mode = B, F, HW, c_latent, c_pad, cfg_dup, mask_frames, _dt(x), mode
        self._call("fyc_unet_input", a)

    def cfg_ddim_step(self, pred: Tensor, latents: Tensor, coef: Tensor, *, B: int, F: int, HW: int, c_latent: int,
                      ld: int, cfg: bool, guidance: float, pred_type: int, clip_sample: bool,
                      pred_single: Optional[Tensor] = None, video_scale: float = 0.0, variance_noise: Optional[Tensor] = None,
                      sigma: float = 0.0, clipped_model_output: bool = False) -> None:
        a = L.CfgDdimArgs()
        if variance_noise is not None and variance_noise.numel() != latents.numel():
            raise ValueError("cfg_ddim_step: variance_noise must have the latents' shape")
        a.variance_noise, a.sigma, a.clipped_model_output = _f32(variance_noise, "variance_noise"), float(sigma), int(clipped_model_output)
        if pred_single is not None and pred_single.dtype != pred.dtype:
            raise TypeError("cfg_ddim_step: pred_single dtype differs from pred")
        a.pred_single, a.video_scale = _p(pred_single), video_scale
        a.pred, a.latents, a.coef = _p(pred), _f32(latents, "latents"), _f32(coef, "coef")
        a.B, a.F, a.HW, a.c_latent, a.ld, a.cfg, a.guidance = B, F, HW, c_latent, ld, int(cfg), guidance
        a.pred_type, a.clip_sample, a.dtype = pred_type, int(clip_sample), _dt(pred)
        self._call("fyc_cfg_ddim_step", a)

    def nchw_to_nhwc(self, z: Tensor, x: Tensor, *, N: int, C_: int, HW: int, c_pad: int, scale: float) -> None:
        self.ensure_init(z.device)
        a = L.NchwInArgs()
        a.z, a.x, a.N, a.C, a.HW, a.c_pad, a.scale, a.dtype = _f32(z, "z"), _p(x), N, C_, HW, c_pad, scale, _dt(x)
        self._call("fyc_nchw_to_nhwc", a)

    def nhwc_to_nchw(self, x: Tensor, y: Tensor, *, N: int, C_: int, HW: int, ld: int, mul: float = 1.0, add: float = 0.0,
                     lo: float = -3.0e38, hi: float = 3.0e38) -> None:
        a = L.NhwcOutArgs()
        a.x, a.y, a.N, a.C, a.HW, a.ld, a.mul, a.add, a.lo, a.hi, a.dtype = _p(x), _f32(y, "y"), N, C_, HW, ld, mul, add, lo, hi, _dt(x)
        self._call("fyc_nhwc_to_nchw", a)


impl = None


def get() -> HipOps:
    global impl
    if impl is None:
        impl = HipOps()
    return impl
```

### followyourclick_amd/profiling.py

```python
from __future__ import annotations

from collections import defaultdict
from typing import Dict

import torch


def _esize(t) -> int:
    return t.element_size()


class TimedOps:
    def __init__(self, inner):
        self.inner = inner
        self.name = inner.name
        self.records = []
        self.enabled = True

    def ensure_init(self, device):
        return self.inner.ensure_init(device)

    def set_tuning(self, key, value):
        return self.inner.set_tuning(key, value)

    def device_caps(self):
        return self.inner.device_caps()

    def _timed(self, family: str, flops: float, nbytes: float, fn, *a, _key=None, **kw):
        if not self.enabled:
            return fn(*a, **kw)
        s, e = torch.cuda.Event(enable_timing=True), torch.cuda.Event(enable_timing=True)
        s.record()
        r = fn(*a, **kw)
        e.record()
        self.records.append((family, s, e, flops, nbytes, _key))
        return r

    def gemm(self, a, w, out, **kw):
        M, N, K, batch = kw["M"], kw["N"], kw["K"], kw.get("batch", 1)
        flops = 2.0 * M * N * K * batch
        es = _esize(a)
        mode = kw.get("mode", 0)
        if mode == 0:
            in_bytes = M * K * es * batch
            fam = "gemm"
        else:
            c = kw["conv"]
            frames = M // (c["Hout"] * c["Wout"])
            in_bytes = frames * c["Hin"] * c["Win"] * c["Cin"] * es
            fam = "conv3x3"
        out_cols = N // 2 if kw.get("epilogue", 0) == 1 else N
        nbytes = in_bytes + N * K * es * batch + M * out_cols * es * batch
        if kw.get("residual") is not None:
            nbytes += M * N * es
        key = f"{fam} M={M} N={N} K={K} b={batch} epi={kw.get('epilogue', 0)} res={int(kw.get('residual') is not None)}"
        return self._timed(fam, flops, nbytes, self.inner.gemm, a, w, out, _key=key, **kw)

    def attention(self, q, k, vt, o, **kw):
        B, H, nq, nk, d = kw["batch"], kw["heads"], kw["n_q"], kw["n_k"], kw["d"]
        flops = 4.0 * B * H * nq * nk * d
        kvb = (B + kw.get("kv_batch_div", 1) - 1) // kw.get("kv_batch_div", 1)
        nbytes = (2 * B * H * nq * d + 2 * kvb * H * nk * d) * 2
        fam = "attn_self" if nq == nk else "attn_cross"
        return self._timed(fam, flops, nbytes, self.inner.attention, q, k, vt, o, _key=f"{fam} B={B} H={H} nq={nq} nk={nk} d={d}", **kw)

    def temporal_attention(self, qkv, o, **kw):
        n = kw["clips"] * kw["frames"] * kw["pixels"] * kw["heads"] * kw["d"]
        flops = 4.0 * kw["clips"] * kw["pixels"] * kw["heads"] * kw["frames"] ** 2 * kw["d"]
        return self._timed("attn_temporal", flops, 4.0 * n * _esize(qkv), self.inner.temporal_attention, qkv, o, **kw)

    def gn_stats(self, x, stats, **kw):
        return self._timed("gn_stats", 0.0, kw["rows"] * kw["C_"] * _esize(x), self.inner.gn_stats, x, stats, **kw)

    def gn_apply(self, x, stats, g, b, y, **kw):
        return self._timed("gn_apply", 0.0, 2.0 * kw["rows"] * kw["C_"] * _esize(x), self.inner.gn_apply, x, stats, g, b, y, **kw)

    def gn_apply_cs(self, x1, cs1, g, b, y, **kw):
        return self._timed("gn_apply", 0.0, 2.0 * kw["rows"] * (kw["C1"] + kw.get("C2", 0)) * _esize(x1), self.inner.gn_apply_cs, x1, cs1, g, b, y, **kw)

    def gemm_row_parts(self, dtype, **kw):
        return self.inner.gemm_row_parts(dtype, **kw)

    def gemm_stat_layout(self, dtype, **kw):
        return self.inner.gemm_stat_layout(dtype, **kw)

    def gemm_split_bytes(self, dtype, **kw):
        return self.inner.gemm_split_bytes(dtype, **kw)

    def temporal_block_supported(self, dtype, **kw):
        return self.inner.temporal_block_supported(dtype, **kw)

    def temporal_block(self, x, out, **kw):
        rows, C = kw["clips"] * kw["frames"] * kw["pixels"], kw["heads"] * kw["d"]
        return self._timed("temporal_block", 2.0 * rows * C * 4 * C + 4.0 * rows * kw["frames"] * C, 2.0 * rows * C * _esize(x),
                           self.inner.temporal_block, x, out, **kw)

    def ff_block_supported(self, dtype, **kw):
        return self.inner.ff_block_supported(dtype, **kw)

    def ff_block(self, x, residual, out, **kw):
        rows, C, hid = kw["rows"], kw["C_"], kw["hidden"]
        flops = 2.0 * rows * (C * 2 * hid + (C + hid) * C)
        nbytes = (2 + (residual is not None)) * rows * C * _esize(x) + (C * 2 * hid + (C + hid) * C) * _esize(x)
        return self._timed("ff_block", flops, nbytes, self.inner.ff_block, x, residual, out, **kw)

    def panel_linear_supported(self, dtype, **kw):
        return self.inner.panel_linear_supported(dtype, **kw)

    def panel_linear(self, x, out, **kw):
        rows, N, K = kw["rows"], kw["N"], kw["K"]
        nbytes = (rows * K + rows * N * (2 if kw.get("residual") is not None else 1) + N * K) * _esize(x)
        key = f"panel_linear M={rows} N={N} K={K} gn={int(kw.get('gn_cs') is not None)} res={int(kw.get('residual') is not None)}"
        return self._timed("panel_linear", 2.0 * rows * N * K, nbytes, self.inner.panel_linear, x, out, _key=key, **kw)

    def chan_stats_reduce(self, parts, cs, **kw):
        return self._timed("gn_stats", 0.0, 0.0, self.inner.chan_stats_reduce, parts, cs, **kw)

    def layernorm(self, x, g, b, y, **kw):
        return self._timed("layernorm", 0.0, 2.0 * kw["rows"] * kw["C_"] * _esize(x), self.inner.layernorm, x, g, b, y, **kw)

    def softmax_rows(self, x, **kw):
        return self._timed("softmax", 0.0, 2.0 * kw["rows"] * kw["cols"] * _esize(x), self.inner.softmax_rows, x, **kw)

    def concat_channels(self, a, b, y, **kw):
        return self._timed("concat", 0.0, 2.0 * kw["rows"] * (kw["c1"] + kw["c2"]) * _esize(a), self.inner.concat_channels, a, b, y, **kw)

    def __getattr__(self, name):
        fn = getattr(self.inner, name)
        if not callable(fn):
            return fn

        def wrapper(*a, **kw):
            return self._timed(name, 0.0, 0.0, fn, *a, **kw)
        return wrapper

    def reset(self):
        self.records = []

    def by_shape(self):
        out = defaultdict(lambda: [0, 0.0, 0.0])
        for fam, s, e, fl, nb, key in self.records:
            d = out[key or fam]
            d[0] += 1
            d[1] += s.elapsed_time(e)
            d[2] += fl
        rows = [(k, v[0], v[1], (v[2] / (v[1] * 1e-3) / 1e12) if v[1] > 0 and v[2] > 0 else 0.0) for k, v in out.items()]
        return sorted(rows, key=lambda r: -r[2])

    def summary(self) -> Dict[str, dict]:
        out = defaultdict(lambda: dict(launches=0, ms=0.0, flops=0.0, bytes=0.0))
        for fam, s, e, fl, nb, _ in self.records:
            d = out[fam]
            d["launches"] += 1
            d["ms"] += s.elapsed_time(e)
            d["flops"] += fl
            d["bytes"] += nb
        return dict(out)
```

### include/fyc.h

```cpp
#ifndef FYC_H
#define FYC_H
#include <stddef.h>
#include <stdint.h>

#ifdef __cplusplus
extern "C" {
#endif

#define FYC_VERSION 301

typedef enum { FYC_F32 = 0, FYC_BF16 = 1, FYC_F16 = 2 } fyc_dtype;

int fyc_version(void);
const char* fyc_last_error(void);
int fyc_init(const void* zero_page);
int fyc_device_caps(int64_t* caps);
int fyc_set_tuning(int key, int value);

enum { FYC_GEMM_PLAIN = 0, FYC_GEMM_CONV3X3 = 1, FYC_GEMM_CONV3X3_UP2 = 2 };
enum { FYC_EPI_LINEAR = 0, FYC_EPI_GEGLU = 1, FYC_EPI_HEADS = 2 };
enum { FYC_ACT_NONE = 0, FYC_ACT_GELU = 1, FYC_ACT_QUICK_GELU = 2 };

typedef struct {
  const void* a;
  const void* a2;
  const void* w;
  const float* bias;
  const float* rowbias;
  const void* residual;
  void* out;
  void* seg_out[3];
  int32_t seg_transposed[3];
  int32_t seg_ld[3];
  int32_t M, N, K;
  int32_t lda, ldw, ldo, ldr;
  int32_t ldrb;
  int32_t k_split, lda2;
  int64_t stride_a, stride_w, stride_o;
  int32_t batch;
  int32_t mode;
  int32_t epilogue;
  int32_t Hout, Wout, Hin, Win, Cin, conv_stride;
  int32_t conv_pad;
  int32_t rows_per_batch;
  int32_t seg_cols, heads, tokens;
  float out_scale;
  int32_t dtype;
  int32_t tile;
  int32_t act;
  const float* ln_stats;
  const float* ln_colsum;
  int32_t ln_nparts; float ln_eps;
  float* chan_parts; int32_t cs_rows;
  float* row_parts; int32_t row_nparts;
  void* workspace; int64_t workspace_bytes;
} fyc_gemm_args;
int fyc_gemm(const fyc_gemm_args* a, void* stream);
int64_t fyc_gemm_workspace_bytes(const fyc_gemm_args* a);
int fyc_gemm_row_parts(const fyc_gemm_args* a);
int fyc_gemm_stat_layout(const fyc_gemm_args* a, int32_t* tile_rows, int32_t* slots);

typedef struct { const float* parts; double* cs; int32_t rows, N, cs_rows, tile_rows, slots, out_rows; } fyc_chan_stats_reduce_args;
int fyc_chan_stats_reduce(const fyc_chan_stats_reduce_args* a, void* stream);

typedef struct {
  const void* q; const void* k; const void* vt; void* o;
  int32_t batch, heads, n_q, n_k, d;
  int32_t ldo;
  int32_t ldvt;
  int32_t kv_batch_div;
  int32_t o_accumulate;
  float scale, o_scale;
  int32_t dtype;
} fyc_attn_args;
int fyc_attention(const fyc_attn_args* a, void* stream);

typedef struct {
  const void* qkv; void* o;
  int32_t clips, frames, pixels, heads, d;
  float scale;
  int32_t dtype;
} fyc_tattn_args;
int fyc_temporal_attention(const fyc_tattn_args* a, void* stream);

typedef struct {
  const void* x; double* stats;
  int32_t rows, C, groups, rows_per_sample;
  int32_t dtype;
  int32_t pad_;
  float* workspace; int64_t workspace_bytes;
} fyc_gn_stats_args;
int fyc_gn_stats(const fyc_gn_stats_args* a, void* stream);
int64_t fyc_gn_stats_workspace(const fyc_gn_stats_args* a);

typedef struct {
  const void* x; const double* stats; const float* gamma; const float* beta; void* y;
  int32_t rows, C, groups, rows_per_sample;
  float eps; int32_t silu;
  int32_t dtype;
} fyc_gn_apply_args;
int fyc_gn_apply(const fyc_gn_apply_args* a, void* stream);

typedef struct {
  const void* x1; const double* cs1; const void* x2; const double* cs2;
  const float* gamma; const float* beta; void* y;
  int32_t C1, C2, rows, groups, rows_per_sample;
  float eps; int32_t silu;
  int32_t dtype;
  int32_t cs_rows;
} fyc_gn_apply_cs_args;
int fyc_gn_apply_cs(const fyc_gn_apply_cs_args* a, void* stream);

typedef struct {
  const void* x; const float* gamma; const float* beta; const float* pe; void* y;
  int32_t rows, C; float eps;
  int32_t pe_div, pe_rows;
  int32_t dtype;
} fyc_layernorm_args;
int fyc_layernorm(const fyc_layernorm_args* a, void* stream);

typedef struct { const void* x; float* stats; int32_t rows, C; float eps; int32_t dtype; } fyc_row_stats_args;
int fyc_row_stats(const fyc_row_stats_args* a, void* stream);

typedef struct { void* x; int64_t rows; int32_t cols, ld; int32_t dtype; int32_t causal_rows; } fyc_softmax_args;
int fyc_softmax_rows(const fyc_softmax_args* a, void* stream);

typedef struct { const void* a; const void* b; void* y; int64_t rows; int32_t c1, c2; int32_t dtype; } fyc_concat_args;
int fyc_concat_channels(const fyc_concat_args* a, void* stream);

typedef struct { const float* x; float* y; int64_t n; } fyc_silu_args;
int fyc_silu_f32(const fyc_silu_args* a, void* stream);

typedef struct { const float* x; void* y; int64_t rows; int32_t cols, ld; int32_t dtype; } fyc_cast_args;
int fyc_cast_from_f32(const fyc_cast_args* a, void* stream);
typedef struct { const void* x; float* y; int64_t rows; int32_t cols, ld; int32_t dtype; } fyc_cast_to_args;
int fyc_cast_to_f32(const fyc_cast_to_args* a, void* stream);

typedef struct {
  const float* latents; const float* mask; const float* first; void* x;
  int32_t B, F, HW, c_latent, c_pad, cfg_dup, mask_frames;
  int32_t dtype;
  int32_t mode;
} fyc_unet_input_args;
int fyc_unet_input(const fyc_unet_input_args* a, void* stream);

typedef struct {
  const void* pred; float* latents; const float* coef;
  int32_t B, F, HW, c_latent, ld, cfg; float guidance;
  int32_t pred_type, clip_sample;
  int32_t dtype;
  const void* pred_single; float video_scale;
  const float* variance_noise; float sigma; int32_t clipped_model_output;
} fyc_cfg_ddim_args;
int fyc_cfg_ddim_step(const fyc_cfg_ddim_args* a, void* stream);

typedef struct { const float* z; void* x; int32_t N, C, HW, c_pad; float scale; int32_t dtype; } fyc_nchw_in_args;
int fyc_nchw_to_nhwc(const fyc_nchw_in_args* a, void* stream);
typedef struct { const void* x; float* y; int32_t N, C, HW, ld; float mul, add, lo, hi; int32_t dtype; } fyc_nhwc_out_args;
int fyc_nhwc_to_nchw(const fyc_nhwc_out_args* a, void* stream);

typedef struct { const int64_t* ids; const float* table; const float* pos; void* out; int64_t rows; int32_t seq, C, vocab; int32_t dtype; } fyc_embed_args;
int fyc_embed_tokens(const fyc_embed_args* a, void* stream);

typedef struct { const float* image; void* out; int32_t B, Cin, H, W, P, ld; int32_t dtype; } fyc_patchify_args;
int fyc_patchify(const fyc_patchify_args* a, void* stream);

typedef struct {
  const void* x; void* out;
  const void* w_qkv; const float* colsum; const float* bias; const float* pe_bias;
  const void* w_out; const float* b_out;
  int32_t clips, frames, pixels, heads, d, C;
  float scale, eps;
  int32_t dtype;
  const void* wstream;
} fyc_temporal_block_args;
int fyc_temporal_block(const fyc_temporal_block_args* a, void* stream);
int64_t fyc_temporal_block_wstream_bytes(void);
int fyc_temporal_block_supported(const fyc_temporal_block_args* a);

typedef struct {
  const void* x; const void* residual; void* out;
  const void* wstream; const float* b_out;
  float* chan_parts; int32_t cs_rows;
  int32_t rows, C, hidden;
  float eps;
  int32_t dtype;
} fyc_ff_block_args;
int fyc_ff_block(const fyc_ff_block_args* a, void* stream);
int fyc_ff_block_supported(const fyc_ff_block_args* a);
int64_t fyc_ff_block_wstream_bytes(void);

typedef struct {
  const void* x; const void* residual; void* out;
  const void* wstream; const float* bias;
  const double* gn_cs; const float* gn_gamma; const float* gn_beta;
  int32_t gn_rows_per_sample, gn_stat_samples, gn_groups;
  float gn_eps;
  int32_t rows, N, K;
  int32_t dtype;
} fyc_panel_linear_args;
int fyc_panel_linear(const fyc_panel_linear_args* a, void* stream);
int fyc_panel_linear_supported(const fyc_panel_linear_args* a);
int64_t fyc_panel_linear_wstream_bytes(int32_t N, int32_t K);

typedef struct { const float* w; void* out; int32_t O, I; int32_t dtype; } fyc_pack_conv3x3_args;
int fyc_pack_conv3x3(const fyc_pack_conv3x3_args* a, void* stream);
typedef struct { const float* w; const float* b; void* w_out; float* b_out; int32_t O, I; int32_t dtype; } fyc_pack_geglu_args;
int fyc_pack_geglu(const fyc_pack_geglu_args* a, void* stream);

#ifdef __cplusplus
}
#endif
#endif
```

Baseline: 13.92 frames/s.

## Fuse proj_in/out linear, residual, LayerNorm and QKV projection into panel chain kernel

Adds a persistent panel_chain kernel for C=320 that runs a 320x320 linear (with optional GroupNorm prologue and residual add), writes h, computes per-row LayerNorm stats in registers, and then runs the LN-folded QKV/Q projection with a head-split epilogue. Weights for both GEMMs are streamed through a double-buffered LDS ring fed by direct global-to-LDS loads. This targets the launches and the HBM round trips of the intermediate activations between the linear, the layernorm and the QKV GEMM in the 64x64 transformer blocks. It adds a complex specialized kernel with a custom K-order weight packing, and the fusion is limited to C=320 shapes.

```diff
diff --git a/followyourclick_amd/_build.py b/followyourclick_amd/_build.py
--- a/followyourclick_amd/_build.py
+++ b/followyourclick_amd/_build.py
@@ -10,7 +10,7 @@
 EXTRA = os.environ.get("FYC_BUILD_EXTRA", "").split()
 LIB = os.path.abspath(os.environ.get("FYC_BUILD_LIB") or os.path.join(HERE, "libfyc_hip.so"))
 OBJ = os.path.join(HERE, "_obj") if not (EXTRA or os.environ.get("FYC_BUILD_LIB")) else LIB + ".obj"
-SOURCES = ["api.hip", "gemm.hip", "gemm_bf16_plain.hip", "gemm_bf16_conv.hip", "gemm_bf16_act.hip", "gemm_f16_plain.hip", "gemm_f16_conv.hip", "gemm_f16_act.hip", "gemm_f32.hip", "attention.hip", "attention_small.hip", "attention_medium.hip", "attention_large.hip", "attention_small_f16.hip", "attention_medium_f16.hip", "attention_large_f16.hip", "temporal_attn.hip", "temporal_block.hip", "temporal_block_rr.hip", "ff_block.hip", "panel_linear.hip", "norm.hip", "elementwise.hip"]
+SOURCES = ["api.hip", "gemm.hip", "gemm_bf16_plain.hip", "gemm_bf16_conv.hip", "gemm_bf16_act.hip", "gemm_f16_plain.hip", "gemm_f16_conv.hip", "gemm_f16_act.hip", "gemm_f32.hip", "attention.hip", "attention_small.hip", "attention_medium.hip", "attention_large.hip", "attention_small_f16.hip", "attention_medium_f16.hip", "attention_large_f16.hip", "temporal_attn.hip", "temporal_block.hip", "temporal_block_rr.hip", "ff_block.hip", "panel_linear.hip", "panel_chain.hip", "norm.hip", "elementwise.hip"]
 VARIANTS = os.environ.get("FYC_GEMM_VARIANTS") == "1"
 VARIANT_DIR = os.path.join(HERE, "..", "tools", "exp", "gemm_variants")
 VARIANT_SOURCES = ["gemm_pp_plain.hip", "gemm_pp_conv.hip", "gemm_ov.hip"] if VARIANTS else []
@@ -20,7 +20,7 @@
         raise SystemExit("FYC_GEMM_VARIANTS=1 needs FYC_BUILD_LIB=<path>: the experiment kernels are not part of the product library")
 FLAGS = ["--offload-arch=gfx950", "-O3", "-std=c++17", "-fPIC", "-ffp-contract=off", "-Wno-unused-value",
          "-mllvm", "-amdgpu-mfma-vgpr-form=1"]
-AGPR_SOURCES = {"ff_block.hip", "panel_linear.hip", "temporal_block_rr.hip"}
+AGPR_SOURCES = {"ff_block.hip", "panel_linear.hip", "panel_chain.hip", "temporal_block_rr.hip"}
 
 
 NO_SLP_SOURCES = set(filter(None, os.environ.get("FYC_NO_SLP", "ff_block.hip").split(",")))
diff --git a/followyourclick_amd/_lib.py b/followyourclick_amd/_lib.py
--- a/followyourclick_amd/_lib.py
+++ b/followyourclick_amd/_lib.py
@@ -132,6 +132,13 @@
                 ("rows", i32), ("N", i32), ("K", i32), ("dtype", i32)]
 
 
+class PanelChainArgs(C.Structure):
+    _fields_ = [("x", vp), ("residual", vp), ("h", vp), ("wstream", vp), ("bias1", vp), ("gn_cs", vp), ("gn_gamma", vp), ("gn_beta", vp),
+                ("gn_rows_per_sample", i32), ("gn_stat_samples", i32), ("gn_groups", i32), ("gn_eps", C.c_float),
+                ("bias2", vp), ("ln_colsum", vp), ("seg_out", vp * 3),
+                ("rows", i32), ("C", i32), ("N2", i32), ("heads", i32), ("tokens", i32), ("ln_eps", C.c_float), ("dtype", i32)]
+
+
 class PackConv3x3Args(C.Structure):
     _fields_ = [("w", vp), ("out", vp), ("O", i32), ("I", i32), ("dtype", i32)]
 
@@ -149,13 +156,14 @@
     "fyc_embed_tokens": EmbedArgs, "fyc_patchify": PatchifyArgs, "fyc_row_stats": RowStatsArgs,
     "fyc_gn_apply_cs": GnApplyCsArgs, "fyc_chan_stats_reduce": ChanStatsReduceArgs,
     "fyc_pack_conv3x3": PackConv3x3Args, "fyc_pack_geglu": PackGegluArgs, "fyc_temporal_block": TemporalBlockArgs,
-    "fyc_ff_block": FFBlockArgs, "fyc_panel_linear": PanelLinearArgs,
+    "fyc_ff_block": FFBlockArgs, "fyc_panel_linear": PanelLinearArgs, "fyc_panel_chain": PanelChainArgs,
 }
 MISC = ["fyc_version", "fyc_last_error", "fyc_init", "fyc_device_caps", "fyc_set_tuning", "fyc_gemm_row_parts", "fyc_gemm_stat_layout", "fyc_gemm_workspace_bytes", "fyc_gn_stats_workspace", "fyc_temporal_block_supported", "fyc_temporal_block_wstream_bytes",
-        "fyc_ff_block_supported", "fyc_ff_block_wstream_bytes", "fyc_panel_linear_supported", "fyc_panel_linear_wstream_bytes"]
+        "fyc_ff_block_supported", "fyc_ff_block_wstream_bytes", "fyc_panel_linear_supported", "fyc_panel_linear_wstream_bytes",
+        "fyc_panel_chain_supported", "fyc_panel_chain_wstream_bytes"]
 
 _lib = None
-FYC_VERSION = 301
+FYC_VERSION = 302
 
 
 class FycError(RuntimeError):
@@ -205,6 +213,11 @@
         lib.fyc_panel_linear_supported.restype = C.c_int
         lib.fyc_panel_linear_wstream_bytes.argtypes = [i32, i32]
         lib.fyc_panel_linear_wstream_bytes.restype = i64
+    if not ab_build or hasattr(lib, "fyc_panel_chain_supported"):
+        lib.fyc_panel_chain_supported.argtypes = [C.POINTER(PanelChainArgs)]
+        lib.fyc_panel_chain_supported.restype = C.c_int
+        lib.fyc_panel_chain_wstream_bytes.argtypes = [i32, i32]
+        lib.fyc_panel_chain_wstream_bytes.restype = i64
     for name, st in OPS.items():
         if ab_build and not hasattr(lib, name):
             continue
diff --git a/followyourclick_amd/csrc/panel_chain.hip b/followyourclick_amd/csrc/panel_chain.hip
--- /dev/null
+++ b/followyourclick_amd/csrc/panel_chain.hip
@@ -0,0 +1,447 @@
+#include <mutex>
+#include <type_traits>
+
+#include "fyc_common.h"
+
+namespace {
+
+constexpr int ROWS = 128, NT = 256, PN = 320, CC = 320;
+constexpr int HEADS = 8, HD = CC / HEADS;
+constexpr int KS = CC / 32;
+constexpr int SPP = KS / 2;
+constexpr int NB = PN / 16;
+constexpr int PIECE = 1024;
+constexpr int NPIECE = 2 * NB;
+constexpr int STAGE_BYTES = NPIECE * PIECE;
+constexpr int RING_BYTES = 2 * STAGE_BYTES;
+constexpr int TILE_BYTES = ROWS * PN * 2;
+constexpr int LDS_BYTES = RING_BYTES + TILE_BYTES;
+static_assert(LDS_BYTES <= 160 * 1024, "LDS budget");
+
+struct PCP {
+  const bf16_t* x; const bf16_t* res; bf16_t* h;
+  const char* ws;
+  const float* b1;
+  const double* gn_cs;
+  const float* gn_gamma; const float* gn_beta;
+  int gn_rows_per_sample, gn_stat_samples, gn_groups;
+  float gn_eps;
+  const float* b2; const float* colsum;
+  bf16_t* seg[3];
+  int tokens;
+  float ln_eps;
+  int npanels;
+};
+
+__device__ __forceinline__ void dma16(const char* gbase, unsigned voff, unsigned lds_dst) {
+  unsigned keep;
+  asm volatile("s_mov_b32 %0, m0\n\ts_mov_b32 m0, %3\n\ts_nop 0\n\tglobal_load_lds_dwordx4 %1, %2\n\ts_mov_b32 m0, %0"
+               : "=&s"(keep) : "v"(voff), "s"(gbase), "s"(lds_dst) : "memory");
+}
+__device__ __forceinline__ void dma16v(const void* gsrc, unsigned lds_dst) {
+  unsigned keep;
+  asm volatile("s_mov_b32 %0, m0\n\ts_mov_b32 m0, %2\n\ts_nop 0\n\tglobal_load_lds_dwordx4 %1, off\n\ts_mov_b32 m0, %0"
+               : "=&s"(keep) : "v"(gsrc), "s"(lds_dst) : "memory");
+}
+__device__ __forceinline__ void dma_landed_barrier() {
+  asm volatile("s_waitcnt vmcnt(0)" ::: "memory");
+  __syncthreads();
+}
+__device__ __forceinline__ f32x4 mfma(bf16x8 a, bf16x8 b, f32x4 c) { return __builtin_amdgcn_mfma_f32_16x16x32_bf16(a, b, c, 0, 0, 0); }
+__device__ __forceinline__ f32x4 mfma(f16x8 a, f16x8 b, f32x4 c) { return __builtin_amdgcn_mfma_f32_16x16x32_f16(a, b, c, 0, 0, 0); }
+template <typename Frag> __device__ __forceinline__ Frag frag(const char* sl, int piece) { return *reinterpret_cast<const Frag*>(sl + piece * PIECE); }
+
+template <typename E16, int NP2>
+__global__ void __launch_bounds__(NT) panel_chain_kernel(const PCP p) {
+  typedef typename Pair16<E16>::Vec8 Frag;
+  constexpr int NST = (1 + NP2) * SPP;
+  static_assert(NST % 2 == 0, "ring parity");
+  extern __shared__ __attribute__((aligned(16))) char smem[];
+  char* const tile = smem + RING_BYTES;
+  const int tid = threadIdx.x, lane = tid & 63;
+  const int wave = __builtin_amdgcn_readfirstlane(tid >> 6);
+  const int g = lane >> 4, r16 = lane & 15;
+  const unsigned lane16 = (unsigned)lane * 16u;
+  const unsigned lds0 = (unsigned)(size_t)(__attribute__((address_space(3))) char*)smem;
+
+  auto dma_piece = [&](const char* ws, unsigned lds, int T, int n) __attribute__((always_inline)) {
+    const int q = wave + 4 * n;
+    dma16(ws + (long long)T * STAGE_BYTES, lane16 + q * PIECE, lds + (T & 1) * STAGE_BYTES + q * PIECE);
+  };
+  Frag xa[2][KS];
+  auto load_x = [&](long long r0) __attribute__((always_inline)) {
+    int rl = r16, gl = g;
+    asm volatile("" : "+v"(rl), "+v"(gl));
+    const bf16_t* xr = p.x + (r0 + wave * 32 + rl) * CC + gl * 8;
+#pragma unroll
+    for (int i = 0; i < 2; ++i)
+#pragma unroll
+      for (int s = 0; s < KS; ++s) xa[i][s] = *reinterpret_cast<const Frag*>(xr + (long long)i * 16 * CC + s * 32);
+  };
+
+  int panel = blockIdx.x;
+  if (panel >= p.npanels) return;
+  load_x((long long)panel * ROWS);
+#pragma unroll
+  for (int n = 0; n < 10; ++n) dma_piece(p.ws, lds0, 0, n);
+
+  for (; panel < p.npanels; panel += gridDim.x) {
+    const long long row0 = (long long)panel * ROWS;
+    const bool has_next = panel + (int)gridDim.x < p.npanels;
+
+    if (p.gn_cs != nullptr) {
+      __syncthreads();
+      double* dsum = reinterpret_cast<double*>(tile);
+      float* tab = reinterpret_cast<float*>(tile + CC * 16);
+      const int sample = (int)(row0 / p.gn_rows_per_sample), cpg = CC / p.gn_groups;
+      int tg = tid;
+      asm volatile("" : "+v"(tg));
+      for (int c = tg; c < CC; c += NT) {
+        double s = 0.0, q = 0.0;
+        for (int f = 0; f < p.gn_stat_samples; ++f) {
+          const double* src = p.gn_cs + (((long long)sample * p.gn_stat_samples + f) * CC + c) * 2;
+          s += src[0]; q += src[1];
+        }
+        dsum[2 * c] = s; dsum[2 * c + 1] = q;
+      }
+      __syncthreads();
+      for (int c = tg; c < CC; c += NT) {
+        const int c0 = (c / cpg) * cpg;
+        double s = 0.0, q = 0.0;
+        for (int j = 0; j < cpg; ++j) { s += dsum[2 * (c0 + j)]; q += dsum[2 * (c0 + j) + 1]; }
+        const double inv_cnt = 1.0 / ((double)p.gn_rows_per_sample * cpg);
+        const double mean = s * inv_cnt;
+        double var = q * inv_cnt - mean * mean;
+        var = var > 0.0 ? var : 0.0;
+        const float rstd = (float)(1.0 / sqrt(var + (double)p.gn_eps));
+        const float sc = rstd * p.gn_gamma[c];
+        tab[2 * c] = sc;
+        tab[2 * c + 1] = p.gn_beta[c] - (float)mean * sc;
+      }
+      __syncthreads();
+#pragma unroll
+      for (int s = 0; s < KS; ++s) {
+        float sc[8], sh[8];
+#pragma unroll
+        for (int e = 0; e < 8; e += 2) {
+          const f32x4 t = *reinterpret_cast<const f32x4*>(tab + 2 * (32 * s + 8 * g + e));
+          sc[e] = t[0]; sh[e] = t[1]; sc[e + 1] = t[2]; sh[e + 1] = t[3];
+        }
+#pragma unroll
+        for (int i = 0; i < 2; ++i) {
+          u32x4 t = __builtin_bit_cast(u32x4, xa[i][s]);
+#pragma unroll
+          for (int e = 0; e < 4; ++e)
+            t[e] = Pair16<E16>::pack(__builtin_fmaf(Pair16<E16>::lo(t[e]), sc[2 * e], sh[2 * e]),
+                                   __builtin_fmaf(Pair16<E16>::hi(t[e]), sc[2 * e + 1], sh[2 * e + 1]));
+          xa[i][s] = __builtin_bit_cast(Frag, t);
+        }
+      }
+      __syncthreads();
+    }
+
+    f32x4 oacc[2][NB];
+    u32x4 hu[2][KS];
+    float mean[2], rstd[2];
+
+    auto stage = [&](const int T, const int st, const bool S2, const bool TR) __attribute__((always_inline)) {
+      const char* sl = smem + (T & 1) * STAGE_BYTES + lane16;
+      long long hide = 0;
+      unsigned lds = lds0;
+      asm volatile("" : "+s"(hide), "+s"(lds));
+      const char* ws = p.ws + hide;
+      Frag wf[2][4];
+#pragma unroll
+      for (int e = 0; e < 4; ++e) wf[0][e] = frag<Frag>(sl, e);
+#pragma unroll
+      for (int grp = 0; grp < 2 * NB / 4; ++grp) {
+        if (grp + 1 < 2 * NB / 4) {
+#pragma unroll
+          for (int e = 0; e < 4; ++e) wf[(grp + 1) & 1][e] = frag<Frag>(sl, 4 * (grp + 1) + e);
+        }
+#pragma unroll
+        for (int e = 0; e < 4; ++e) {
+          const int u = 4 * grp + e, sk = u / NB, j = u % NB;
+#pragma unroll
+          for (int i = 0; i < 2; ++i) {
+            const Frag op = S2 ? __builtin_bit_cast(Frag, hu[i][2 * st + sk]) : xa[i][2 * st + sk];
+            oacc[i][j] = TR ? mfma(op, wf[grp & 1][e], oacc[i][j]) : mfma(wf[grp & 1][e], op, oacc[i][j]);
+          }
+          if (u < 10) {
+            if (T + 1 < NST) dma_piece(ws, lds, T + 1, u);
+            else if (has_next) dma_piece(ws, lds, 0, u);
+          }
+        }
+        __builtin_amdgcn_sched_barrier(0);
+      }
+    };
+    auto zero_acc = [&]() __attribute__((always_inline)) {
+#pragma unroll
+      for (int i = 0; i < 2; ++i)
+#pragma unroll
+        for (int j = 0; j < NB; ++j) oacc[i][j] = (f32x4){0.f, 0.f, 0.f, 0.f};
+    };
+
+    constexpr int VG = 2;
+    f32x4 bv[2][VG], cv[2][VG];
+    auto ld_vec = [&](const float* b, const float* c, int grp, int slot) __attribute__((always_inline)) {
+#pragma unroll
+      for (int e = 0; e < VG; ++e) {
+        bv[slot][e] = b != nullptr ? *reinterpret_cast<const f32x4*>(b + (VG * grp + e) * 16 + g * 4) : (f32x4){0.f, 0.f, 0.f, 0.f};
+        if (c != nullptr) cv[slot][e] = *reinterpret_cast<const f32x4*>(c + (VG * grp + e) * 16 + g * 4);
+      }
+    };
+    long long hide1 = 0;
+    asm volatile("" : "+s"(hide1));
+    const float* b1 = p.b1 != nullptr ? p.b1 + hide1 : nullptr;
+    zero_acc();
+#pragma unroll
+    for (int st = 0; st < SPP; ++st) {
+      dma_landed_barrier();
+      if (st == SPP - 1 && p.res != nullptr) {
+        const bf16_t* rbase = p.res + row0 * CC;
+        int ln = lane;
+        asm volatile("" : "+v"(ln));
+#pragma unroll
+        for (int n = 0; n < TILE_BYTES / PIECE / 4; ++n) {
+          const int c = (wave + 4 * n) * 64 + ln, row = c / 40, cg = c - row * 40;
+          dma16(reinterpret_cast<const char*>(rbase), (unsigned)(row * CC + cg * 8) * 2u, lds0 + RING_BYTES + (wave + 4 * n) * PIECE);
+        }
+      }
+      if (st == SPP - 1) ld_vec(b1, nullptr, 0, 0);
+      stage(st, st, false, false);
+    }
+    dma_landed_barrier();
+#pragma unroll
+    for (int grp = 0; grp < NB / VG; ++grp) {
+      if (grp + 1 < NB / VG) ld_vec(b1, nullptr, grp + 1, (grp + 1) & 1);
+#pragma unroll
+      for (int e = 0; e < VG; ++e)
+#pragma unroll
+        for (int i = 0; i < 2; ++i) {
+          const int j = VG * grp + e;
+          E16* a = reinterpret_cast<E16*>(tile + (wave * 32 + i * 16 + r16) * (PN * 2)) + j * 16 + g * 4;
+          const f32x4 bo = bv[grp & 1][e];
+          float rr[4] = {0.f, 0.f, 0.f, 0.f}, v[4];
+          if (p.res != nullptr) ElemIO<E16>::ld4(a, rr);
+#pragma unroll
+          for (int r = 0; r < 4; ++r) v[r] = oacc[i][j][r] + bo[r] + rr[r];
+          u32x2 t;
+          t[0] = Pair16<E16>::pack(v[0], v[1]);
+          t[1] = Pair16<E16>::pack(v[2], v[3]);
+          *reinterpret_cast<u32x2*>(a) = t;
+          hu[i][j / 2][2 * (j & 1)] = t[0];
+          hu[i][j / 2][2 * (j & 1) + 1] = t[1];
+        }
+      __builtin_amdgcn_sched_barrier(0);
+    }
+    __syncthreads();
+    {
+      int tl = tid;
+      asm volatile("" : "+v"(tl));
+      const int cg = tl % 40, rsl = tl / 40;
+      if (rsl < 6) {
+        char* dst = reinterpret_cast<char*>(p.h + row0 * CC) + cg * 16;
+        const char* src = tile + cg * 16;
+#pragma unroll 2
+        for (int row = rsl; row < ROWS; row += 6)
+          *reinterpret_cast<u32x4*>(dst + (long long)row * CC * 2) = *reinterpret_cast<const u32x4*>(src + row * (PN * 2));
+      }
+    }
+#pragma unroll
+    for (int i = 0; i < 2; ++i) {
+      float s = 0.f;
+#pragma unroll
+      for (int k = 0; k < KS; ++k)
+#pragma unroll
+        for (int e = 0; e < 4; ++e) s += Pair16<E16>::lo(hu[i][k][e]) + Pair16<E16>::hi(hu[i][k][e]);
+      s = swap32_sum(swap16_sum(s));
+      const float m = s / (float)CC;
+      float q = 0.f;
+#pragma unroll
+      for (int k = 0; k < KS; ++k) asm volatile("" : "+v"(hu[i][k]));
+#pragma unroll
+      for (int k = 0; k < KS; ++k)
+#pragma unroll
+        for (int e = 0; e < 4; ++e) {
+          const float d0 = Pair16<E16>::lo(hu[i][k][e]) - m, d1 = Pair16<E16>::hi(hu[i][k][e]) - m;
+          q += d0 * d0;
+          q += d1 * d1;
+        }
+      q = swap32_sum(swap16_sum(q));
+      mean[i] = m;
+      rstd[i] = rsqrtf(q / (float)CC + p.ln_eps);
+    }
+
+    const int bf = (int)(row0 / p.tokens), t0 = (int)(row0 - (long long)bf * p.tokens);
+    auto do_pass = [&](auto pass_c) __attribute__((always_inline)) {
+      constexpr int pass = decltype(pass_c)::value;
+      constexpr bool TR = pass == 2;
+      long long hide2 = pass * PN;
+      int r16l = r16;
+      asm volatile("" : "+s"(hide2), "+v"(r16l));
+      const float* cs = p.colsum + hide2;
+      const float* b2 = p.b2 != nullptr ? p.b2 + hide2 : nullptr;
+      zero_acc();
+#pragma unroll
+      for (int st = 0; st < SPP; ++st) {
+        dma_landed_barrier();
+        if (!TR && st == SPP - 1) ld_vec(b2, cs, 0, 0);
+        stage((1 + pass) * SPP + st, st, true, TR);
+      }
+      if constexpr (!TR) {
+#pragma unroll
+        for (int grp = 0; grp < NB / VG; ++grp) {
+          if (grp + 1 < NB / VG) ld_vec(b2, cs, grp + 1, (grp + 1) & 1);
+#pragma unroll
+          for (int e = 0; e < VG; ++e)
+#pragma unroll
+            for (int i = 0; i < 2; ++i) {
+              const int j = VG * grp + e;
+              E16* a = reinterpret_cast<E16*>(tile + (wave * 32 + i * 16 + r16) * (PN * 2)) + j * 16 + g * 4;
+              const f32x4 c4 = cv[grp & 1][e], bo = bv[grp & 1][e];
+              float v[4];
+#pragma unroll
+              for (int r = 0; r < 4; ++r) v[r] = rstd[i] * (oacc[i][j][r] - mean[i] * c4[r]) + bo[r];
+              ElemIO<E16>::st4(a, v);
+            }
+          __builtin_amdgcn_sched_barrier(0);
+        }
+        if (pass == NP2 - 1 && has_next) load_x(row0 + (long long)gridDim.x * ROWS);
+        __syncthreads();
+        constexpr int dch = HD / 8, per_head = ROWS * dch;
+        char* const seg = reinterpret_cast<char*>(p.seg[pass]) + (((long long)bf * HEADS * p.tokens + t0) * HD << 1);
+        int tl = tid;
+        asm volatile("" : "+v"(tl));
+#pragma unroll 4
+        for (int n = 0; n < ROWS * PN * 2 / 16 / NT; ++n) {
+          const int c = tl + NT * n, head = c / per_head, within = c - head * per_head, row = within / dch, part = within - row * dch;
+          const u32x4 v = *reinterpret_cast<const u32x4*>(tile + row * (PN * 2) + head * (HD * 2) + part * 16);
+          *reinterpret_cast<u32x4*>(seg + ((long long)head * p.tokens * HD << 1) + within * 16) = v;
+        }
+      } else {
+        float mt[2][4], rt[2][4];
+#pragma unroll
+        for (int i = 0; i < 2; ++i)
+#pragma unroll
+          for (int r = 0; r < 4; ++r) {
+            float m4[4], r4[4];
+#pragma unroll
+            for (int gg = 0; gg < 4; ++gg) {
+              m4[gg] = __uint_as_float(__builtin_amdgcn_readlane(__float_as_uint(mean[i]), 4 * gg + r));
+              r4[gg] = __uint_as_float(__builtin_amdgcn_readlane(__float_as_uint(rstd[i]), 4 * gg + r));
+            }
+            mt[i][r] = g == 0 ? m4[0] : g == 1 ? m4[1] : g == 2 ? m4[2] : m4[3];
+            rt[i][r] = g == 0 ? r4[0] : g == 1 ? r4[1] : g == 2 ? r4[2] : r4[3];
+          }
+#pragma unroll
+        for (int j = 0; j < NB; ++j) {
+          const int f = j * 16 + r16l;
+          const float c1 = cs[f], bo = b2 != nullptr ? b2[f] : 0.f;
+#pragma unroll
+          for (int i = 0; i < 2; ++i) {
+            float v[4];
+#pragma unroll
+            for (int r = 0; r < 4; ++r) v[r] = rt[i][r] * (oacc[i][j][r] - mt[i][r] * c1) + bo;
+            const int unit = (wave * 8 + i * 4 + g) ^ (r16l << 1);
+            ElemIO<E16>::st4(reinterpret_cast<E16*>(tile + f * 256 + unit * 8), v);
+          }
+          if ((j & 3) == 3) __builtin_amdgcn_sched_barrier(0);
+        }
+        if (pass == NP2 - 1 && has_next) load_x(row0 + (long long)gridDim.x * ROWS);
+        __syncthreads();
+        char* const seg = reinterpret_cast<char*>(p.seg[2]) + (((long long)bf * PN * p.tokens + t0) << 1);
+        int tl = tid;
+        asm volatile("" : "+v"(tl));
+#pragma unroll 4
+        for (int n = 0; n < ROWS * PN * 2 / 16 / NT; ++n) {
+          const int c = tl + NT * n, f = c >> 4, ch = c & 15;
+          const u32x4 v = *reinterpret_cast<const u32x4*>(tile + f * 256 + ((ch ^ (f & 15)) << 4));
+          *reinterpret_cast<u32x4*>(seg + ((long long)f * p.tokens << 1) + ch * 16) = v;
+        }
+      }
+    };
+    do_pass(std::integral_constant<int, 0>{});
+    if constexpr (NP2 == 3) {
+      do_pass(std::integral_constant<int, 1>{});
+      do_pass(std::integral_constant<int, 2>{});
+    }
+  }
+}
+
+template <typename T, int NP2>
+int launch(const PCP& p, hipStream_t st) {
+  auto kern = panel_chain_kernel<T, NP2>;
+  int64_t caps[8];
+  {
+    constexpr int kMaxDev = 64;
+    static std::mutex mu;
+    static bool attr_done[kMaxDev] = {};
+    static int64_t cus[kMaxDev] = {};
+    int dev = 0;
+    (void)hipGetDevice(&dev);
+    std::lock_guard<std::mutex> lk(mu);
+    if (dev < 0 || dev >= kMaxDev || !attr_done[dev]) {
+      const hipError_t e = hipFuncSetAttribute(reinterpret_cast<const void*>(kern), hipFuncAttributeMaxDynamicSharedMemorySize, LDS_BYTES);
+      if (e != hipSuccess) FYC_FAIL(-3, "fyc_panel_chain: %d bytes of dynamic LDS refused: %s", LDS_BYTES, hipGetErrorString(e));
+      if (fyc_device_caps(caps) != 0) return -3;
+      if (dev >= 0 && dev < kMaxDev) { attr_done[dev] = true; cus[dev] = caps[0]; }
+    } else {
+      caps[0] = cus[dev];
+    }
+  }
+  const int grid = (int)(caps[0] > 0 && caps[0] < p.npanels ? caps[0] : p.npanels);
+  hipLaunchKernelGGL(kern, dim3((unsigned)grid), dim3(NT), LDS_BYTES, st, p);
+  FYC_CHECK_LAUNCH("fyc_panel_chain");
+  return 0;
+}
+
+}
+
+extern "C" int64_t fyc_panel_chain_wstream_bytes(int32_t C, int32_t N2) {
+  if (C != CC || N2 <= 0 || N2 % PN != 0) return 0;
+  return (int64_t)(1 + N2 / PN) * SPP * STAGE_BYTES;
+}
+
+extern "C" int fyc_panel_chain_supported(const fyc_panel_chain_args* a) {
+  if (a == nullptr || (a->dtype != FYC_BF16 && a->dtype != FYC_F16) || a->rows <= 0 || a->rows % ROWS != 0) return 0;
+  if (a->C != CC || (a->N2 != CC && a->N2 != 3 * CC)) return 0;
+  if (a->tokens <= 0 || a->tokens % ROWS != 0 || a->rows % a->tokens != 0) return 0;
+  if (a->heads != HEADS) return 0;
+  if (a->gn_cs != nullptr && (a->gn_rows_per_sample <= 0 || a->gn_rows_per_sample % ROWS != 0 || a->rows % a->gn_rows_per_sample != 0 ||
+                              a->gn_groups <= 0 || a->C % a->gn_groups != 0 || a->gn_stat_samples <= 0)) return 0;
+  static std::mutex mu;
+  static int64_t lds_cap = -1;
+  {
+    std::lock_guard<std::mutex> lk(mu);
+    if (lds_cap < 0) {
+      int64_t caps[8];
+      lds_cap = (fyc_device_caps(caps) == 0) ? caps[1] : 0;
+    }
+  }
+  return (lds_cap > 0 && lds_cap < LDS_BYTES) ? 0 : 1;
+}
+
+extern "C" int fyc_panel_chain(const fyc_panel_chain_args* a, void* stream) {
+  FYC_REQUIRE(a && a->x && a->h && a->wstream && a->ln_colsum && a->seg_out[0], "fyc_panel_chain: null pointer");
+  FYC_REQUIRE(fyc_panel_chain_supported(a), "fyc_panel_chain: built for bf16 / f16, C = 320, N2 in {320, 960}, tokens %% 128 == 0, 8 heads, "
+              "GroupNorm samples of whole 128-row tiles (got rows=%d C=%d N2=%d tokens=%d heads=%d gn_rows_per_sample=%d)",
+              a->rows, a->C, a->N2, a->tokens, a->heads, a->gn_rows_per_sample);
+  FYC_REQUIRE(a->N2 == CC || (a->seg_out[1] != nullptr && a->seg_out[2] != nullptr), "fyc_panel_chain: N2 = 3C needs seg_out[0..2] (q, k, V^T)");
+  FYC_REQUIRE(a->gn_cs == nullptr || (a->gn_gamma != nullptr && a->gn_beta != nullptr), "fyc_panel_chain: gn_cs needs gn_gamma / gn_beta");
+  FYC_REQUIRE(a->x != a->h && a->residual != a->x, "fyc_panel_chain: h must not alias x (residual may alias h)");
+  FYC_REQUIRE(((uintptr_t)a->x % 16) == 0 && ((uintptr_t)a->h % 16) == 0 && ((uintptr_t)a->wstream % 16) == 0 && ((uintptr_t)a->bias1 % 16) == 0 &&
+              ((uintptr_t)a->residual % 16) == 0 && ((uintptr_t)a->gn_cs % 16) == 0 && ((uintptr_t)a->bias2 % 16) == 0 && ((uintptr_t)a->ln_colsum % 16) == 0 &&
+              ((uintptr_t)a->seg_out[0] % 16) == 0 && ((uintptr_t)a->seg_out[1] % 16) == 0 && ((uintptr_t)a->seg_out[2] % 16) == 0,
+              "fyc_panel_chain: operands must be 16-byte aligned");
+  PCP p;
+  p.x = (const bf16_t*)a->x; p.res = (const bf16_t*)a->residual; p.h = (bf16_t*)a->h; p.ws = (const char*)a->wstream; p.b1 = a->bias1;
+  p.gn_cs = a->gn_cs; p.gn_gamma = a->gn_gamma; p.gn_beta = a->gn_beta; p.gn_rows_per_sample = a->gn_rows_per_sample;
+  p.gn_stat_samples = a->gn_stat_samples; p.gn_groups = a->gn_groups; p.gn_eps = a->gn_eps;
+  p.b2 = a->bias2; p.colsum = a->ln_colsum;
+  for (int i = 0; i < 3; ++i) p.seg[i] = (bf16_t*)a->seg_out[i];
+  p.tokens = a->tokens; p.ln_eps = a->ln_eps; p.npanels = a->rows / ROWS;
+  hipStream_t st = (hipStream_t)stream;
+  if (a->dtype == FYC_F16) return a->N2 == CC ? launch<f16_t, 1>(p, st) : launch<f16_t, 3>(p, st);
+  return a->N2 == CC ? launch<bf16_t, 1>(p, st) : launch<bf16_t, 3>(p, st);
+}
diff --git a/followyourclick_amd/engine/unet3d.py b/followyourclick_amd/engine/unet3d.py
--- a/followyourclick_amd/engine/unet3d.py
+++ b/followyourclick_amd/engine/unet3d.py
@@ -10,7 +10,7 @@
 from .. import ops as ops_mod
 from .base import EngineBase
 from .config import UNet3DConfig
-from .weights import Packed, pack_ff_block, pack_panel_linear, pack_temporal_block
+from .weights import Packed, pack_ff_block, pack_panel_chain, pack_panel_linear, pack_temporal_block
 
 Tensor = torch.Tensor
 
@@ -20,6 +20,7 @@
 FUSE_FF = os.environ.get("FYC_FUSE_FF", "1") != "0"
 FUSE_PANEL = os.environ.get("FYC_FUSE_PANEL", "1") != "0"
 PANEL_ALL = os.environ.get("FYC_PANEL_ALL", "0") != "0"
+FUSE_CHAIN = os.environ.get("FYC_FUSE_CHAIN", "1") != "0"
 FUSE_ROWS = os.environ.get("FYC_FUSE_ROWS", "0") != "0"
 
 
@@ -207,6 +208,19 @@
             return Act(out, C)
         h, _ = self._gn(x, node.norm_g, node.norm_b, rows, rows_per_sample, 1e-6, False)
         return self._lin_rp(h, node.pin_w, rows, bias=node.pin_b)
+
+    def _chain_ok(self, rows: int, C: int, N2: int, tokens: int, folded, gn_rows_per_sample: int = 0) -> bool:
+        sup = getattr(self.ops, "panel_chain_supported", None)
+        if not (FUSE_CHAIN and FUSE_PANEL) or sup is None or folded is None or self.fuse_rows:
+            return False
+        return sup(self.dtype, rows=rows, C_=C, N2=N2, heads=self.heads, tokens=tokens, gn_rows_per_sample=gn_rows_per_sample, gn_groups=self.groups)
+
+    def _chain_stream(self, t: Packed, name: str, w1: Tensor, w2: Tensor) -> Tensor:
+        key = "_chain_" + name
+        hit = t.get(key)
+        if hit is None or hit[0] is not w1 or hit[1] is not w2:
+            hit = t[key] = (w1, w2, pack_panel_chain(w1, w2))
+        return hit[2]
 
     def _ln_args(self, tok: Act, rows: int, C: int) -> dict:
         if tok.rp is not None:
@@ -300,29 +314,44 @@
         rows, C, H, o = g["rows"], t.C, self.heads, self.ops
         BF, N = g["B"] * g["F"], g["H"] * g["W"]
         d = C // H
-        tok = self._norm_proj_in(x, t, rows, N)
         ld = ((N + 7) // 8) * 8
         q, k, vt = self.new(BF, H, N, d), self.new(BF, H, N, d), (self.zeros(BF, H, d, ld) if ld != N else self.new(BF, H, d, ld))
         hd = dict(seg_cols=C, heads=H, tokens=N, outs=[q, k, vt], transposed=[0, 0, 1], ld=[0, 0, ld])
-        if t.qkv_f is not None:
+        if (isinstance(x, Act) and x.cs is not None and N % x.cs_rows == 0
+                and self._chain_ok(rows, C, 3 * C, N, t.qkv_f, gn_rows_per_sample=N)):
             w, b, cs = t.qkv_f
-            o.gemm(tok.t, w, None, M=rows, N=3 * C, K=C, lda=C, ldw=C, bias=b, epilogue=L.EPI_HEADS, heads=hd, ln_colsum=cs,
-                   **self._ln_args(tok, rows, C))
+            tok = Act(self.new(rows, C), C)
+            o.panel_chain(x.t, tok.t, [q, k, vt], wstream=self._chain_stream(t, "front", t.pin_w, w), rows=rows, C_=C, N2=3 * C, heads=H,
+                          tokens=N, bias1=t.pin_b, bias2=b, ln_colsum=cs, ln_eps=1e-5, gn_cs=x.cs, gn_gamma=t.norm_g, gn_beta=t.norm_b,
+                          gn_rows_per_sample=N, gn_stat_samples=N // x.cs_rows, gn_groups=self.groups, gn_eps=1e-6)
         else:
-            n1 = self.layer_norm(tok.t, t.ln1, rows, C)
-            o.gemm(n1, t.qkv_w, None, M=rows, N=3 * C, K=C, lda=C, ldw=C, epilogue=L.EPI_HEADS, heads=hd)
+            tok = self._norm_proj_in(x, t, rows, N)
+            if t.qkv_f is not None:
+                w, b, cs = t.qkv_f
+                o.gemm(tok.t, w, None, M=rows, N=3 * C, K=C, lda=C, ldw=C, bias=b, epilogue=L.EPI_HEADS, heads=hd, ln_colsum=cs,
+                       **self._ln_args(tok, rows, C))
+            else:
+                n1 = self.layer_norm(tok.t, t.ln1, rows, C)
+                o.gemm(n1, t.qkv_w, None, M=rows, N=3 * C, K=C, lda=C, ldw=C, epilogue=L.EPI_HEADS, heads=hd)
         att = self.new(rows, C)
         self._attend(q, k, vt, att, batch=BF, n_q=N, n_k=N, d=d, ldvt=ld, C=C, kv_div=1)
-        tok = self._lin_rp(att, t.o1_w, rows, bias=t.o1_b, residual=tok.t)
         q2 = self.new(BF, H, N, d)
         hd2 = dict(seg_cols=C, heads=H, tokens=N, outs=[q2], transposed=[0], ld=[0])
-        if t.q2_f is not None:
+        if self._chain_ok(rows, C, C, N, t.q2_f):
             w, b, cs = t.q2_f
-            o.gemm(tok.t, w, None, M=rows, N=C, K=C, lda=C, ldw=C, bias=b, epilogue=L.EPI_HEADS, heads=hd2, ln_colsum=cs,
-                   **self._ln_args(tok, rows, C))
+            nxt_tok = Act(self.new(rows, C), C)
+            o.panel_chain(att, nxt_tok.t, [q2], wstream=self._chain_stream(t, "middle", t.o1_w, w), rows=rows, C_=C, N2=C, heads=H,
+                          tokens=N, bias1=t.o1_b, residual=tok.t, bias2=b, ln_colsum=cs, ln_eps=1e-5)
+            tok = nxt_tok
         else:
-            n2 = self.layer_norm(tok.t, t.ln2, rows, C)
-            o.gemm(n2, t.q2_w, None, M=rows, N=C, K=C, lda=C, ldw=C, epilogue=L.EPI_HEADS, heads=hd2)
+            tok = self._lin_rp(att, t.o1_w, rows, bias=t.o1_b, residual=tok.t)
+            if t.q2_f is not None:
+                w, b, cs = t.q2_f
+                o.gemm(tok.t, w, None, M=rows, N=C, K=C, lda=C, ldw=C, bias=b, epilogue=L.EPI_HEADS, heads=hd2, ln_colsum=cs,
+                       **self._ln_args(tok, rows, C))
+            else:
+                n2 = self.layer_norm(tok.t, t.ln2, rows, C)
+                o.gemm(n2, t.q2_w, None, M=rows, N=C, K=C, lda=C, ldw=C, epilogue=L.EPI_HEADS, heads=hd2)
         cache = self.ctx_cache[t.idx]
         kt, vtt, ldt = cache["text"]
         att2 = self.new(rows, C)
diff --git a/followyourclick_amd/engine/weights.py b/followyourclick_amd/engine/weights.py
--- a/followyourclick_amd/engine/weights.py
+++ b/followyourclick_amd/engine/weights.py
@@ -286,6 +286,34 @@
     assert N % pn == 0 and pn % 16 == 0 and K % 64 == 0
     fr = _mfma_fragments(w.reshape(N // pn, pn // 16, 16, K // 64, 2, 32).permute(0, 3, 4, 1, 2, 5))
     return fr.reshape(-1).contiguous()
+
+
+def panel_chain_korder(K: int) -> Tensor:
+    slot = torch.arange(32)
+    g, e = slot // 8, slot % 8
+    within = 16 * (e // 4) + 4 * g + e % 4
+    return (torch.arange(K // 32)[:, None] * 32 + within[None, :]).reshape(-1)
+
+
+def pack_panel_chain(w1: Tensor, w2_folded: Tensor) -> Tensor:
+    C = w1.shape[1]
+    assert tuple(w1.shape) == (C, C) and w2_folded.shape[1] == C and w1.dtype == w2_folded.dtype
+    order = panel_chain_korder(C).to(w2_folded.device)
+    return torch.cat([pack_panel_linear(w1), pack_panel_linear(w2_folded[:, order].contiguous())]).contiguous()
+
+
+def unpack_panel_chain(stream: Tensor, C: int, N2: int):
+    def unpack(fr: Tensor, N: int) -> Tensor:
+        pn_ = min(N, 320)
+        blocks = fr.reshape(N // pn_, C // 64, 2, pn_ // 16, 4, 16, 8).transpose(-3, -2)
+        return blocks.reshape(N // pn_, C // 64, 2, pn_ // 16, 16, 32).permute(0, 3, 4, 1, 2, 5).reshape(N, C)
+
+    n1 = C * C
+    w1 = unpack(stream[:n1], C)
+    w2p = unpack(stream[n1:], N2)
+    w2 = torch.empty_like(w2p)
+    w2[:, panel_chain_korder(C).to(w2p.device)] = w2p
+    return w1, w2
 
 
 def sinusoidal_pe(channels: int, length: int) -> Tensor:
diff --git a/followyourclick_amd/ops.py b/followyourclick_amd/ops.py
--- a/followyourclick_amd/ops.py
+++ b/followyourclick_amd/ops.py
@@ -3,7 +3,7 @@
 import os
 
 import ctypes as C
-from typing import Optional
+from typing import Optional, Sequence
 
 import torch
 
@@ -294,6 +294,50 @@
         a.rows, a.N, a.K, a.dtype = rows, N, K, _dt(x)
         self._call("fyc_panel_linear", a)
 
+    def panel_chain_supported(self, dtype: torch.dtype, *, rows: int, C_: int, N2: int, heads: int, tokens: int,
+                              gn_rows_per_sample: int = 0, gn_groups: int = 32) -> bool:
+        if not hasattr(self.lib, "fyc_panel_chain_supported"):
+            return False
+        key = ("pcs", dtype, rows, C_, N2, heads, tokens, gn_rows_per_sample, gn_groups)
+        if key not in self._q_cache:
+            a = L.PanelChainArgs()
+            a.rows, a.C, a.N2, a.heads, a.tokens = rows, C_, N2, heads, tokens
+            a.dtype = _dtc(dtype)
+            if gn_rows_per_sample > 0:
+                a.gn_cs, a.gn_rows_per_sample, a.gn_stat_samples, a.gn_groups = 16, gn_rows_per_sample, 1, gn_groups
+            self._q_cache[key] = bool(self.lib.fyc_panel_chain_supported(C.byref(a)))
+        return self._q_cache[key]
+
+    def panel_chain(self, x: Tensor, h: Tensor, outs: Sequence[Tensor], *, wstream: Tensor, rows: int, C_: int, N2: int, heads: int,
+                    tokens: int, bias2: Optional[Tensor], ln_colsum: Tensor, bias1: Optional[Tensor] = None,
+                    residual: Optional[Tensor] = None, ln_eps: float = 1e-5, gn_cs: Optional[Tensor] = None,
+                    gn_gamma: Optional[Tensor] = None, gn_beta: Optional[Tensor] = None, gn_rows_per_sample: int = 0,
+                    gn_stat_samples: int = 1, gn_groups: int = 32, gn_eps: float = 1e-6) -> None:
+        self.ensure_init(x.device)
+        key = ("pcw", C_, N2)
+        if key not in self._q_cache:
+            self._q_cache[key] = int(self.lib.fyc_panel_chain_wstream_bytes(C_, N2))
+        need = self._q_cache[key]
+        if wstream.numel() * wstream.element_size() != need:
+            raise ValueError(f"panel_chain: wstream has {wstream.numel() * wstream.element_size()} bytes, expected {need}")
+        if gn_cs is not None and gn_cs.dtype != torch.float64:
+            raise TypeError("panel_chain: gn_cs must be float64")
+        if len(outs) != N2 // C_:
+            raise ValueError(f"panel_chain: {len(outs)} output segments for N2 = {N2}, C = {C_}")
+        frames = rows // tokens
+        for t in outs:
+            if t.dtype != x.dtype or t.numel() != frames * tokens * C_ or not t.is_contiguous():
+                raise ValueError("panel_chain: every output segment is a contiguous [frames][heads][...] tensor of rows * C elements of x's dtype")
+        a = L.PanelChainArgs()
+        a.x, a.residual, a.h, a.wstream, a.bias1 = _p(x), _p(residual), _p(h), _p(wstream), _f32(bias1, "bias1")
+        a.gn_cs, a.gn_gamma, a.gn_beta = _p(gn_cs), _f32(gn_gamma, "gn_gamma"), _f32(gn_beta, "gn_beta")
+        a.gn_rows_per_sample, a.gn_stat_samples, a.gn_groups, a.gn_eps = gn_rows_per_sample, gn_stat_samples, gn_groups, gn_eps
+        a.bias2, a.ln_colsum = _f32(bias2, "bias2"), _f32(ln_colsum, "ln_colsum")
+        for i, t in enumerate(outs):
+            a.seg_out[i] = _p(t)
+        a.rows, a.C, a.N2, a.heads, a.tokens, a.ln_eps, a.dtype = rows, C_, N2, heads, tokens, ln_eps, _dt(x)
+        self._call("fyc_panel_chain", a)
+
     def gn_stats(self, x: Tensor, stats: Tensor, *, rows: int, C_: int, groups: int, rows_per_sample: int) -> None:
         a = L.GnStatsArgs()
         if stats.dtype != torch.float64:
diff --git a/followyourclick_amd/profiling.py b/followyourclick_amd/profiling.py
--- a/followyourclick_amd/profiling.py
+++ b/followyourclick_amd/profiling.py
@@ -113,6 +113,19 @@
         key = f"panel_linear M={rows} N={N} K={K} gn={int(kw.get('gn_cs') is not None)} res={int(kw.get('residual') is not None)}"
         return self._timed("panel_linear", 2.0 * rows * N * K, nbytes, self.inner.panel_linear, x, out, _key=key, **kw)
 
+    def panel_chain_supported(self, dtype, **kw):
+        return self.inner.panel_chain_supported(dtype, **kw)
+
+    def panel_chain(self, x, h, outs, **kw):
+        rows, C, N2 = kw["rows"], kw["C_"], kw["N2"]
+        nbytes = (rows * C * (2 + (kw.get("residual") is not None)) + rows * N2 + C * (C + N2)) * _esize(x)
+        key = f"panel_chain M={rows} C={C} N2={N2} gn={int(kw.get('gn_cs') is not None)} res={int(kw.get('residual') is not None)}"
+        return self._timed("panel_chain", 2.0 * rows * C * (C + N2), nbytes, self.inner.panel_chain, x, h, outs, _key=key, **kw)
+
+    def row_stats(self, x, stats, **kw):
+        return self._timed("row_stats", 0.0, kw["rows"] * kw["C_"] * _esize(x), self.inner.row_stats, x, stats,
+                           _key=f"row_stats M={kw['rows']} C={kw['C_']}", **kw)
+
     def chan_stats_reduce(self, parts, cs, **kw):
         return self._timed("gn_stats", 0.0, 0.0, self.inner.chan_stats_reduce, parts, cs, **kw)
 
diff --git a/include/fyc.h b/include/fyc.h
--- a/include/fyc.h
+++ b/include/fyc.h
@@ -7,7 +7,7 @@
 extern "C" {
 #endif
 
-#define FYC_VERSION 301
+#define FYC_VERSION 302
 
 typedef enum { FYC_F32 = 0, FYC_BF16 = 1, FYC_F16 = 2 } fyc_dtype;
 
@@ -203,6 +203,22 @@
 int fyc_panel_linear_supported(const fyc_panel_linear_args* a);
 int64_t fyc_panel_linear_wstream_bytes(int32_t N, int32_t K);
 
+typedef struct {
+  const void* x; const void* residual; void* h;
+  const void* wstream; const float* bias1;
+  const double* gn_cs; const float* gn_gamma; const float* gn_beta;
+  int32_t gn_rows_per_sample, gn_stat_samples, gn_groups;
+  float gn_eps;
+  const float* bias2; const float* ln_colsum;
+  void* seg_out[3];
+  int32_t rows, C, N2, heads, tokens;
+  float ln_eps;
+  int32_t dtype;
+} fyc_panel_chain_args;
+int fyc_panel_chain(const fyc_panel_chain_args* a, void* stream);
+int fyc_panel_chain_supported(const fyc_panel_chain_args* a);
+int64_t fyc_panel_chain_wstream_bytes(int32_t C, int32_t N2);
+
 typedef struct { const float* w; void* out; int32_t O, I; int32_t dtype; } fyc_pack_conv3x3_args;
 int fyc_pack_conv3x3(const fyc_pack_conv3x3_args* a, void* stream);
 typedef struct { const float* w; const float* b; void* w_out; float* b_out; int32_t O, I; int32_t dtype; } fyc_pack_geglu_args;
```

Result: faster. 14.07 frames/s, median of 6 (+1.1%).
